# robotics-upo/social_force_window_planner

Measured on AMD Instinct MI355X. Metric: scored trajectories/sec (v x w samples x steps) @ N pedestrians; cmd_vel match, higher is better.
Workload: dtype f64

## Files before the change

include/sfw_hip.h:

```cpp
#ifndef SFW_HIP_H_
#define SFW_HIP_H_

#include <stdint.h>

#ifdef __cplusplus
extern "C" {
#endif

#define SFW_ABI_VERSION 2

typedef enum sfw_status {
  SFW_OK = 0,
  SFW_ERR_INVALID_ARG = -1,
  SFW_ERR_NO_DEVICE = -2,
  SFW_ERR_HIP = -3,
  SFW_ERR_STATE = -4,
  SFW_ERR_UNSUPPORTED = -5
} sfw_status;

#define SFW_COST_INVALID (-1.0)
#define SFW_COST_SKIPPED (-2.0)

#define SFW_ROBOT_ID_NONE INT32_MIN

// ... 69 lines not shown
typedef struct sfw_planner_s *sfw_handle;

void sfw_params_default(sfw_params *p);
int sfw_abi_version(void);
int sfw_create(const sfw_params *params, int device, sfw_handle *out);
int sfw_destroy(sfw_handle h);
int sfw_set_params(sfw_handle h, const sfw_params *params);
const char *sfw_last_error(sfw_handle h);

int sfw_set_costmap(sfw_handle h, const uint8_t *cells, uint32_t size_x,
                    uint32_t size_y, double origin_x, double origin_y,
                    double resolution);
int sfw_set_footprint(sfw_handle h, const double *xy, int32_t K);
int sfw_set_agents(sfw_handle h, const sfw_agent *agents, int32_t A,
                   const double *obstacles_xy, int32_t O);

int sfw_score_grid(sfw_handle h, const sfw_robot_state *rs,
                   const double *linvels, int32_t nv, const double *angvels,
                   int32_t nw, const sfw_goal_args *args, double *costs_out,
                   sfw_best *best_out);

int sfw_score_one(sfw_handle h, const sfw_robot_state *rs, double vx_samp,
                  double vy_samp, double vtheta_samp, const sfw_goal_args *args,
                  double *cost_out, double *points_xyth, int32_t points_cap,
                  int32_t *n_points);

int sfw_grid_stage(sfw_handle h, const sfw_robot_state *rs,
                   const double *linvels, int32_t nv, const double *angvels,
                   int32_t nw, const sfw_goal_args *args, int64_t index_base);
int sfw_grid_launch(sfw_handle h);
int sfw_grid_sync(sfw_handle h);
int sfw_grid_fetch(sfw_handle h, double *costs_out, sfw_best *best_out,
                   sfw_best_key *key_out);
const double *sfw_grid_costs_view(sfw_handle h);

int sfw_samples_stage(sfw_handle h, const sfw_robot_state *rs, const double *vx, const double *vy,
                      const double *vtheta, int32_t n, const sfw_goal_args *args, int64_t index_base);
int sfw_score_samples(sfw_handle h, const sfw_robot_state *rs, const double *vx, const double *vy,
                      const double *vtheta, int32_t n, const sfw_goal_args *args, double *costs_out,
                      sfw_best *best_out);

#define SFW_SEQ_MAX_KNOTS 64
int sfw_sequences_stage(sfw_handle h, const sfw_robot_state *rs, const double *vx, const double *vy,
                        const double *vtheta, int32_t n, int32_t K, const int32_t *knot_step,
                        const sfw_goal_args *args, int64_t index_base);
int sfw_score_sequences(sfw_handle h, const sfw_robot_state *rs, const double *vx, const double *vy,
                        const double *vtheta, int32_t n, int32_t K, const int32_t *knot_step,
                        const sfw_goal_args *args, double *costs_out, sfw_best *best_out);

#define SFW_PERTURB_KEEP_NOMINAL 1
#define SFW_PERTURB_NO_VY        2
#define SFW_PERTURB_KEEP_NORMALS 4
typedef struct sfw_perturb {
  uint64_t seed;
  const double *nominal;
  double sigma[3];
  double lo[3], hi[3];
  int32_t flags, reserved;
} sfw_perturb;
int sfw_sequences_perturb_stage(sfw_handle h, const sfw_robot_state *rs, const sfw_perturb *p, int32_t n, int32_t K,
                                const int32_t *knot_step, const sfw_goal_args *args, int64_t index_base);
int sfw_score_perturbed(sfw_handle h, const sfw_robot_state *rs, const sfw_perturb *p, int32_t n, int32_t K,
                        const int32_t *knot_step, const sfw_goal_args *args, double *costs_out, sfw_best *best_out);
int sfw_sequences_knots(sfw_handle h, int64_t first, int64_t count, double *vx_out, double *vy_out, double *vtheta_out);
int sfw_sequences_normals(sfw_handle h, int64_t first, int64_t count, double *z_out);

#define SFW_ORG_NONE 0
#define SFW_ORG_REGISTER_1 1
#define SFW_ORG_REGISTER_2 2
#define SFW_ORG_FLAT 3
typedef struct sfw_plan_info {
  int32_t split_step;
  int32_t levels;
  int32_t chunks;
  int32_t organisation;
  int64_t classes;
  int64_t class_steps;
  int64_t samples;
  int64_t flat_samples;
  int64_t one_launch;
  int64_t rest_noise_unreproduced;
} sfw_plan_info;
int sfw_grid_plan_info(sfw_handle h, sfw_plan_info *out);
int sfw_plan_shared_prefix(const double *linvels, int32_t nv,
                           const double *angvels, int32_t nw, double vx0,
                           double vtheta0, double acc_x, double acc_theta,
                           double sim_time, int32_t num_steps,
                           int32_t n_agents, int32_t *level_ends,
                           int64_t *level_classes, int32_t cap,
                           int32_t *n_levels);
int sfw_plan_axis_classes(const double *targets, int32_t n, double v0, double a_max, double dt, int32_t max_p,
                          int32_t form, int32_t *counts, int32_t *classes, int32_t *n_levels, int32_t *closed_form);
int sfw_plan_row_blocks(const double *linvels, int32_t nv, const double *angvels, int32_t nw, double vx0,
                        double vtheta0, double acc_x, double acc_theta, double sim_time, int32_t num_steps,
                        int32_t n_agents, int32_t R, int32_t *row0);
#define SFW_K2_AUTO (-1)
#define SFW_K2_REGISTER 0
#define SFW_K2_FLAT 1
int sfw_set_k2_form(sfw_handle h, int32_t form);
int sfw_set_timing(sfw_handle h, int32_t enabled);
int sfw_last_launch_ms(sfw_handle h, int32_t which, float *ms_out);
int sfw_last_clock_ghz(sfw_handle h, double *ghz_out);
int sfw_grid_points(sfw_handle h, int64_t index, double *points_xyth,
                    int32_t points_cap, int32_t *n_points);
int sfw_grid_points_batch(sfw_handle h, int64_t first, int64_t count, double *points_xyth, int32_t *n_points);
int sfw_set_points_capture(sfw_handle h, int32_t enabled);
void *sfw_stream(sfw_handle h);

#define SFW_TERM_VEL 0
#define SFW_TERM_DISTANCE 1
#define SFW_TERM_ANGLE 2
#define SFW_TERM_COSTMAP 3
#define SFW_TERM_SOCIAL 4
#define SFW_N_TERMS 5
#define SFW_RESCORE_MAX_K 1024
typedef struct sfw_weights {
  double vel, distance, angle, costmap, social;
} sfw_weights;
int sfw_set_terms_capture(sfw_handle h, int32_t enabled);
int sfw_grid_rescore(sfw_handle h, const sfw_weights *w, int32_t K, sfw_best *best_out, double *costs_out);
int sfw_grid_terms(sfw_handle h, int64_t first, int64_t count, double *terms_out);

#define SFW_BLEND_MAX_L 16
typedef struct sfw_blend_stat {
  double lambda;
  double j_min;
  double eta;
  double sum_w2;
  int64_t n_valid;
  int64_t index_min;
} sfw_blend_stat;
int sfw_grid_blend(sfw_handle h, const double *lambda, int32_t L, const double *bias,
                   sfw_blend_stat *stat_out, double *u_out, double *weights_out);

int sfw_sequences_control_cost(sfw_handle h, double gamma, double *bias_out);
int sfw_grid_blend_control(sfw_handle h, const double *lambda, int32_t L, double gamma, const double *bias,
                           sfw_blend_stat *stat_out, double *u_out, double *weights_out);

#define SFW_MPPI_MAX_ITER 32
typedef struct sfw_mppi {
  int32_t iterations, reserved;
  double lambda;
  double gamma;
} sfw_mppi;
int sfw_mppi_run(sfw_handle h, const sfw_robot_state *rs, const sfw_perturb *p, int32_t n, int32_t K,
                 const int32_t *knot_step, const sfw_goal_args *args, const sfw_mppi *m,
                 sfw_blend_stat *stat_out , double *plans_out , sfw_best *best_out );

int sfw_score_one_crowd(sfw_handle h, const sfw_robot_state *rs, double vx_samp, double vy_samp, double vtheta_samp,
                        const sfw_goal_args *args, double *cost_out, double *state_xyvv, double *work, int32_t *has_goal,
                        int32_t agents, int32_t steps_cap, int32_t *n_steps);
int sfw_grid_crowd(sfw_handle h, int64_t index, double *cost_out, double *state_xyvv, double *work, int32_t *has_goal,
                   int32_t agents, int32_t steps_cap, int32_t *n_steps);

typedef struct sfw_multi_s *sfw_multi_handle;
#define SFW_MULTI_RCCL 0
#define SFW_MULTI_HOST_REDUCE 1
int sfw_multi_create(const sfw_params *params, const int *devices, int32_t R, int32_t exchange,
                     sfw_multi_handle *out);
int sfw_multi_destroy(sfw_multi_handle m);
const char *sfw_multi_last_error(sfw_multi_handle m);
int32_t sfw_multi_ranks(sfw_multi_handle m);
typedef struct sfw_multi_desc {
  int32_t ranks, exchange, communicators, comm_size, rccl_version;
  int32_t devices[64], comm_devices[64];
  char rccl_path[512], rccl_found[64];
// ... 79 lines not shown
```

social_force_window_planner_amd/_abi.py:

```python
import ctypes as C

SFW_OK = 0
SFW_ERR_INVALID_ARG = -1
SFW_ERR_NO_DEVICE = -2
SFW_ERR_HIP = -3
SFW_ERR_STATE = -4
SFW_ERR_UNSUPPORTED = -5

SFW_COST_INVALID = -1.0
SFW_COST_SKIPPED = -2.0

SFW_PRECISION_F64 = 0
SFW_PRECISION_F32 = 1
SFW_PRECISION_F64_STRICT = 2

SFW_K2_AUTO, SFW_K2_REGISTER, SFW_K2_FLAT = -1, 0, 1
SFW_ORG_NONE, SFW_ORG_REGISTER_1, SFW_ORG_REGISTER_2, SFW_ORG_FLAT = 0, 1, 2, 3


class SfwParams(C.Structure):
    _fields_ = [
        ("max_vel_x", C.c_double),
        ("sim_time", C.c_double),
        ("sim_granularity", C.c_double),
# ... 51 lines not shown
        if not hasattr(p, k):
            raise AttributeError(f"sfw_params has no field {k!r}")
        setattr(p, k, v)
    return p


class SfwAgent(C.Structure):
    _fields_ = [
        ("x", C.c_double),
        ("y", C.c_double),
        ("vx", C.c_double),
        ("vy", C.c_double),
        ("goal_x", C.c_double),
        ("goal_y", C.c_double),
        ("goal_radius", C.c_double),
        ("desired_velocity", C.c_double),
        ("radius", C.c_double),
        ("has_goal", C.c_int32),
        ("id", C.c_int32),
        ("group_id", C.c_int32),
        ("reserved", C.c_int32),
    ]


class SfwRobotState(C.Structure):
    _fields_ = [(n, C.c_double) for n in ("x", "y", "theta", "vx", "vy", "vtheta")]


class SfwGoalArgs(C.Structure):
    _fields_ = [(n, C.c_double) for n in ("acc_x", "acc_y", "acc_theta", "wpx", "wpy")]


class SfwBest(C.Structure):
    _fields_ = [
        ("index", C.c_int64),
        ("cost", C.c_double),
        ("vx", C.c_double),
        ("vy", C.c_double),
        ("vtheta", C.c_double),
        ("n_valid", C.c_int64),
    ]

    def as_dict(self):
        return {n: getattr(self, n) for n, _ in self._fields_}


class SfwBestKey(C.Structure):
    _fields_ = [(n, C.c_double) for n in ("cost", "neg_linvel", "abs_angvel", "neg_index")]

    def as_tuple(self):
        return (self.cost, self.neg_linvel, self.abs_angvel, self.neg_index)


class SfwPlanInfo(C.Structure):
    _fields_ = [("split_step", C.c_int32), ("levels", C.c_int32), ("chunks", C.c_int32), ("organisation", C.c_int32),
                ("classes", C.c_int64), ("class_steps", C.c_int64), ("samples", C.c_int64), ("flat_samples", C.c_int64),
                ("one_launch", C.c_int64), ("rest_noise_unreproduced", C.c_int64)]

    def as_dict(self):
        return {"split_step": self.split_step, "levels": self.levels, "chunks": self.chunks, "classes": self.classes,
                "class_steps": self.class_steps, "samples": self.samples, "organisation": self.organisation,
                "flat_samples": self.flat_samples, "one_launch": self.one_launch,
                "rest_noise_unreproduced": self.rest_noise_unreproduced}


EXPORTED_SYMBOLS = (
    "sfw_params_default",
    "sfw_abi_version",
    "sfw_create",
    "sfw_destroy",
    "sfw_set_params",
    "sfw_last_error",
    "sfw_set_costmap",
    "sfw_set_footprint",
    "sfw_set_agents",
    "sfw_score_grid",
    "sfw_score_one",
    "sfw_grid_stage",
    "sfw_grid_launch",
    "sfw_grid_sync",
    "sfw_grid_fetch",
    "sfw_grid_costs_view",
    "sfw_grid_plan_info",
    "sfw_plan_shared_prefix",
    "sfw_plan_row_blocks",
    "sfw_plan_axis_classes",
    "sfw_set_k2_form",
    "sfw_set_timing",
    "sfw_last_launch_ms",
    "sfw_last_clock_ghz",
    "sfw_grid_points",
    "sfw_grid_points_batch",
    "sfw_set_points_capture",
    "sfw_stream",
    "sfw_multi_create",
    "sfw_multi_destroy",
    "sfw_multi_last_error",
    "sfw_multi_describe",
    "sfw_multi_ranks",
    "sfw_multi_rank_handle",
    "sfw_multi_set_params",
    "sfw_multi_set_costmap",
    "sfw_multi_set_footprint",
    "sfw_multi_set_agents",
    "sfw_multi_score_grid",
    "sfw_multi_rank_rows",
    "sfw_multi_last_us",
    "sfw_multi_grid_points",
    "sfw_batch_create",
    "sfw_batch_destroy",
    "sfw_batch_last_error",
    "sfw_batch_size",
    "sfw_batch_member",
    "sfw_batch_launch",
    "sfw_batch_fetch",
    "sfw_batch_score_grid",
    "sfw_batch_describe",
    "sfw_batch_last_us",
    "sfw_set_terms_capture",
    "sfw_grid_rescore",
    "sfw_grid_terms",
    "sfw_ensemble_create",
    "sfw_ensemble_destroy",
    "sfw_ensemble_last_error",
    "sfw_ensemble_size",
    "sfw_ensemble_member",
    "sfw_ensemble_set_params",
    "sfw_ensemble_set_costmap",
    "sfw_ensemble_set_footprint",
    "sfw_ensemble_set_hypothesis",
    "sfw_ensemble_score_grid",
    "sfw_ensemble_aggregate",
    "sfw_ensemble_last_us",
    "sfw_samples_stage",
    "sfw_score_samples",
    "sfw_sequences_stage",
    "sfw_score_sequences",
    "sfw_score_one_crowd",
    "sfw_grid_crowd",
    "sfw_grid_blend",
    "sfw_sequences_perturb_stage",
    "sfw_score_perturbed",
    "sfw_sequences_knots",
    "sfw_sequences_normals",
    "sfw_ensemble_score_sequences",
    "sfw_ensemble_score_perturbed",
    "sfw_ensemble_blend",
    "sfw_sequences_control_cost",
    "sfw_grid_blend_control",
    "sfw_mppi_run",
    "sfw_ensemble_blend_control",
    "sfw_ensemble_mppi_run",
)
SFW_TERM_VEL, SFW_TERM_DISTANCE, SFW_TERM_ANGLE, SFW_TERM_COSTMAP, SFW_TERM_SOCIAL = 0, 1, 2, 3, 4
SFW_N_TERMS = 5
SFW_RESCORE_MAX_K = 1024


class SfwWeights(C.Structure):

    _fields_ = [("vel", C.c_double), ("distance", C.c_double), ("angle", C.c_double), ("costmap", C.c_double),
                ("social", C.c_double)]


SFW_BLEND_MAX_L = 16

# ... 74 lines not shown
```

social_force_window_planner_amd/csrc/sfw_capi.hip:

```cpp

#include "sfw_device.h"

#include <dlfcn.h>
#include <link.h>

#include <algorithm>
#include <chrono>
#include <cmath>
#include <condition_variable>
#include <functional>
#include <mutex>
#include <thread>
#include <cstdio>
#include <cstdlib>
#include <cstring>
#include <limits>
#include <new>
#include <string>
#include <vector>

namespace {

template <typename T> struct dev_buf {
  T *p = nullptr;
// ... 8 lines not shown
    cap = 0;
    size_t want = n + n / 8 + 16;
    hipError_t e = hipMalloc(reinterpret_cast<void **>(&p), want * sizeof(T));
    if (e == hipSuccess) cap = want;
    return e;
  }
  void release() {
    if (p) (void)hipFree(p);
    p = nullptr;
    cap = 0;
  }
};

struct pinned_buf {
  char *p = nullptr;
  size_t cap = 0;
  hipEvent_t done = nullptr;
  bool pending = false;
  pinned_buf() = default;
  pinned_buf(const pinned_buf &) = delete;
  pinned_buf &operator=(const pinned_buf &) = delete;
  hipError_t wait() {
    if (!pending) return hipSuccess;
    pending = false;
    return hipEventSynchronize(done);
  }
  hipError_t reserve(size_t bytes) {
    hipError_t e = wait();
    if (e != hipSuccess) return e;
    if (!done && (e = hipEventCreateWithFlags(&done, hipEventDisableTiming)) != hipSuccess) return e;
    if (bytes <= cap) return hipSuccess;
    if (p) (void)hipHostFree(p);
    p = nullptr;
    cap = 0;
    const size_t want = bytes + bytes / 4 + 256;
    e = hipHostMalloc(reinterpret_cast<void **>(&p), want, hipHostMallocDefault);
    if (e == hipSuccess) cap = want;
    return e;
  }
  hipError_t mark(hipStream_t s) {
    pending = true;
    return hipEventRecord(done, s);
  }
  void release() {
    (void)wait();
    if (p) (void)hipHostFree(p);
    if (done) (void)hipEventDestroy(done);
    p = nullptr;
    cap = 0;
    done = nullptr;
  }
};

struct level_tables {
  int32_t n_row = 0, n_col = 0;
  size_t o_row_rep = 0, o_col_rep = 0;
  size_t o_row_src = 0, o_col_src = 0;
};
struct chunk_plan {
  std::vector<level_tables> lv;
  size_t o_row_cls = 0;
};

struct map_geometry {
  uint32_t size_x, size_y;
  double origin_x, origin_y, resolution;
};

struct agent_set {
  std::vector<char> blob;
  size_t ao_vel = 0, ao_cst = 0, ao_obs = 0, ao_grp = 0, ao_off = 0, ao_mem = 0;
  int A = 0, O = 0, NG = 0, n_grp_mem = 0;
  bool person_pinned = false;
  std::vector<std::pair<int32_t, int32_t>> rest_pairs;
};

}

struct sfw_planner_s {
  struct config {
    int n_cu = SFW_DEFAULT_CUS, n_xcd = SFW_DEFAULT_CUS / SFW_CUS_PER_XCD;
    std::vector<int> prefix_env;
    bool pin_rest_on = true;
    long spin_us = 20000;
    bool arena_direct_on = true;
    size_t mirror_max_bytes = size_t(64) << 20;
    int obs_tasks_force = -1;
    size_t table_budget_bytes = size_t(8) << 30;
    bool owns_streams = true;
    bool batch_member = false;
  } cfg;

  struct switches {
    sfw_params params;
    uint64_t params_epoch = 1;
    int k2_form = SFW_K2_AUTO;
    bool timing = false;
    bool capture_points = false;
    bool capture_terms = false;
  } live;

  struct world_state {
    map_geometry map_new{0, 0, 0, 0, 0};
    bool have_costmap = false;
    bool cells_dirty = false;
    std::vector<double> footprint;
    int K = 0;
    agent_set agents;
  } world;

  struct stage_record {
    bool valid = false;
    std::vector<double> lin, ang;
    int nv = 0, nw = 0;
    sfw_robot_state rs{};
    sfw_goal_args ga{};
    double vy_samp = 0.0;
    int skip_zero = 1;
    int64_t index_base = 0;
    bool list = false;
    std::vector<double> vy;
    int nk = 1;
    std::vector<int32_t> knot_step;
    const int32_t *d_knot_step = nullptr;
    bool perturbed = false, zero_admitted = false, normals_kept = false;
    sfw_perturb_dev pert{};
    int K = 0, A = 0, O = 0, NG = 0, n_grp_mem = 0;
    bool person_pinned = false;
    map_geometry map{0, 0, 0, 0, 0};
    const uint8_t *d_cells = nullptr;
    bool cells_in_arena = false;
    size_t arena_cells_bytes = 0;
    const double *d_footprint = nullptr, *d_agent_pos = nullptr, *d_agent_vel = nullptr, *d_obstacles = nullptr;
    const sfw_agent_const *d_agent_c = nullptr;
    const int32_t *d_agent_grp = nullptr, *d_grp_off = nullptr, *d_grp_mem = nullptr;
    const double *d_linvels = nullptr, *d_angvels = nullptr;
    const double *d_vy = nullptr;
    const double *d_agent_rest = nullptr;
    const double *d_pin_rest = nullptr;
    sfw_sel *d_sel = nullptr;
    std::vector<std::pair<int32_t, int32_t>> rest_pairs;
    std::vector<double> rest_pv;
    size_t pin_doubles = 0;
    std::vector<double> pin_pos;
    std::vector<sfw_agent_const> pin_cst;
    std::vector<int> prefix_steps;
    std::vector<chunk_plan> prefix_chunks;
    size_t prefix_o_col_cls = 0;
    int prefix_S = 0;
    int64_t prefix_chunk = 0;
    int64_t prefix_class_steps = 0, prefix_last_classes = 0;
    std::vector<int32_t> cls_ints;
    int64_t cls_max = 0;
    bool cls_two = false;
    const int32_t *d_cls_tab = nullptr;
    int64_t table_chunk = 0;
    uint64_t plan_epoch = 0;
    bool arena_pending = false;
    size_t arena_from = 0, arena_bytes = 0;
    bool early_poses = false;
    bool early_poses_timed = false;
    bool early_poses_terms = false;
    bool clock_cleared = false;
  } st;

  struct launch_record {
// ... 113 lines not shown
        return e;
      }
      polled = true;
      if (std::chrono::duration_cast<std::chrono::microseconds>(std::chrono::steady_clock::now() - t0).count() > h->cfg.spin_us) break;
#if defined(__x86_64__)
      __builtin_ia32_pause();
#endif
    }
    (void)hipGetLastError();
  }
  return hipStreamSynchronize(h->stream);
}
void stream_is_idle(sfw_handle h) { h->pin_map.pending = h->pin_arena.pending = h->pin_cls.pending = false; }

constexpr int64_t kRowLimit = static_cast<int64_t>((uint64_t(1) << 32) / (2 * sizeof(sfw_unit))) - 2;

int num_steps_of(const sfw_params &p) {
  int n = static_cast<int>(p.sim_time / p.sim_granularity + 0.5);
  return n == 0 ? 1 : n;
}

int check_params(sfw_handle h, const sfw_params *p) {
  if (!p) return fail(h, SFW_ERR_INVALID_ARG, "params is NULL");
  if (!(p->sim_granularity > 0) || !(p->sim_time >= 0))
    return fail(h, SFW_ERR_INVALID_ARG, "sim_time/sim_granularity out of range");
  if (p->precision != SFW_PRECISION_F64 && p->precision != SFW_PRECISION_F32 && p->precision != SFW_PRECISION_F64_STRICT)
    return fail(h, SFW_ERR_INVALID_ARG, "unknown precision");
  if (!(p->sfm_gamma > 0) || !(p->sfm_relaxation_time > 0) || !(p->sfm_force_sigma_obstacle > 0))
    return fail(h, SFW_ERR_INVALID_ARG, "sfm gamma/relaxation_time/sigma must be > 0");
  if (!(p->sfm_force_factor_social >= 0) || !(p->sfm_force_factor_obstacle >= 0))
    return fail(h, SFW_ERR_INVALID_ARG, "sfm_force_factor_social / _obstacle must be >= 0");
  return SFW_OK;
}

int64_t table_row_units(int64_t stride, int nw) { return stride + stride / (nw > 0 ? nw : 1) + 2; }
constexpr size_t kTableBytesPerSampleStep = sizeof(sfw_unit) + sizeof(int16_t);

void fill_launch(sfw_handle h, sfw_launch &L, int64_t begin, int64_t count, int64_t stride) {
  std::memset(&L, 0, sizeof(L));
  L.p = h->live.params;
  L.S = num_steps_of(h->live.params);
  L.dt = h->live.params.sim_time / L.S;
  L.rs = h->st.rs;
  L.ga = h->st.ga;
  L.vy_samp = h->st.vy_samp;
  L.skip_zero_sample = h->st.skip_zero;
  L.linvels = h->st.d_linvels;
  L.angvels = h->st.d_angvels;
  L.nv = h->st.nv;
  L.nw = h->st.nw;
  L.vy_samps = h->st.d_vy;
  L.list = h->st.list ? 1 : 0;
  L.n_knots = h->st.nk;
  L.knot_step = h->st.d_knot_step;
  L.knot_stride = h->st.nv;
  L.chunk_begin = begin;
  L.chunk_count = count;
  L.cells = h->st.d_cells;
  L.size_x = h->st.map.size_x;
  L.size_y = h->st.map.size_y;
  L.origin_x = h->st.map.origin_x;
  L.origin_y = h->st.map.origin_y;
  L.resolution = h->st.map.resolution;
  L.footprint = h->st.d_footprint;
  L.K = h->st.K;
  L.agent_pos = h->st.d_agent_pos;
  L.agent_vel = h->st.d_agent_vel;
  L.agent_c = h->st.d_agent_c;
  L.agent_rest = h->st.d_agent_rest;
  L.pin_rest = h->st.d_pin_rest;
  L.A = h->st.A;
  L.obstacles = h->st.d_obstacles;
  L.O = h->st.O;
  L.agent_grp = h->st.d_agent_grp;
  L.grp_off = h->st.d_grp_off;
  L.grp_mem = h->st.d_grp_mem;
  L.NG = h->st.NG;
  L.n_grp_mem = h->st.n_grp_mem;
  L.n_cu = h->cfg.n_cu;
  L.n_xcd = h->cfg.n_xcd;
  sfw_derive(L);
  if (h->cfg.obs_tasks_force >= 0 && L.O > 0) L.k.obs_tasks = h->cfg.obs_tasks_force;
  L.pair_tab = h->pair_tab.p;
  L.status = h->status.p;
  L.base_cost = h->base_cost.p;
  L.costs = h->costs.p;
  L.coll_step = h->coll_step.p;
  L.ptab = h->ptab.p;
  L.cs_tab = h->cs_tab.p;
  L.row_units = table_row_units(stride, h->st.nw);
  L.fcode = h->fcode.p;
  L.rstep_stride = stride;
  L.points = nullptr;
  L.n_points = nullptr;
  L.phase = SFW_PHASE_WHOLE;
  L.step_begin = 0;
  L.step_end = L.S;
  L.resume = 0;
  L.k2_form = h->live.k2_form;
  L.index_base = h->st.index_base;
  L.cycle_counter = h->cycle_counter.p;
  L.sel_out = h->st.d_sel;
  L.costs_host = nullptr;
  L.sel_host = nullptr;
  L.arena_host = nullptr;
  L.arena_dev = nullptr;
  L.arena_bytes = 0;
}

double new_velocity_host(double vg, double vi, double a_max, double dt) {
  if ((vg - vi) >= 0) return std::fmin(vg, vi + a_max * dt);
  return std::fmax(vg, vi - a_max * dt);
}

void velocity_classes(const std::vector<double> &targets, double v0, double a_max, double dt, int max_p,
                      std::vector<std::vector<int32_t>> &cls, std::vector<int32_t> &counts) {
  const size_t n = targets.size();
  std::vector<int32_t> order(n);
  for (size_t i = 0; i < n; ++i) order[i] = static_cast<int32_t>(i);
  std::sort(order.begin(), order.end(), [&](int32_t a, int32_t b) {
    return targets[static_cast<size_t>(a)] != targets[static_cast<size_t>(b)] ? targets[static_cast<size_t>(a)] < targets[static_cast<size_t>(b)]
                                                                                : a < b;
  });
  std::vector<double> t(n), v(n, v0);
  for (size_t k = 0; k < n; ++k) t[k] = targets[static_cast<size_t>(order[k])];
  std::vector<int32_t> cur(n, 0), nxt(n);
  cls.clear();
  counts.clear();
  for (int p = 0; p < max_p; ++p) {
    int32_t id = -1;
    uint64_t prev_bits = 0;
    for (size_t k = 0; k < n; ++k) {
      v[k] = new_velocity_host(t[k], v[k], a_max, dt);
      uint64_t bits;
      std::memcpy(&bits, &v[k], sizeof(bits));
      if (k == 0 || cur[k] != cur[k - 1] || bits != prev_bits) ++id;
      nxt[k] = id;
      prev_bits = bits;
    }
    cur.swap(nxt);
    cls.emplace_back(n);
    std::vector<int32_t> &out = cls.back();
    for (size_t k = 0; k < n; ++k) out[static_cast<size_t>(order[k])] = cur[k];
    counts.push_back(id + 1);
    if (static_cast<size_t>(id + 1) == n) break;
  }
}

double step_cost(double items, double items_per_wave, int cus) {
  const double capacity = 4.0 * cus * 5.5;
  const double x = items / items_per_wave / capacity;
  return x <= 1.0 ? 0.45 + 0.55 * x : x;
}

struct axis_classes {
  std::vector<int32_t> n;
  std::vector<double> targets;
  double v0 = 0, a_max = 0, dt = 0;
  int max_p = 0;
  bool made_for(const std::vector<double> &t, double v0_, double a_, double dt_, int mp) const {
    return v0 == v0_ && a_max == a_ && dt == dt_ && max_p == mp && targets == t;
  }
  const std::vector<int32_t> &level(int p) const {
    const size_t l = std::min<size_t>(static_cast<size_t>(p), n.size()) - 1;
    if (!fast) return c[l];
    if (c[l].empty()) write_level(l);
// ... 1221 lines not shown
                                         const_cast<double *>(h->st.d_angvels), h->st.normals_kept ? h->normals.p : nullptr, h->stream));
    }
    if (int e = launch_common(h)) return e;
    const double *d_bias = nullptr;
    if (m->gamma != 0.0) {
      if (int e = control_cost_enqueue(h, m->gamma, nullptr, plan, h->ctrl_bias, h->blend_bias)) return e;
      d_bias = h->ctrl_bias.p;
    }
    if (int e = blend_enqueue(h, area, h->costs.p, n, K, h->st.d_linvels, h->st.d_vy, h->st.d_angvels, 1, true, &m->lambda, 1, d_bias,
                              nullptr, pin + i * slot, plan))
      return e;
  }
  SFW_HIP(h, h->pin_mppi.mark(h->stream));
  sfw_best best;
  if (int e = sfw_grid_fetch(h, nullptr, &best, nullptr)) return e;
  h->pin_mppi.pending = false;
  for (int i = 0; i < I; ++i) blend_finish(pin + i * slot, &m->lambda, 1, K, stat_out + i, plans_out + static_cast<size_t>(i) * 3 * K);
  if (I > 1) std::memcpy(h->st.pert.nominal, plans_out + static_cast<size_t>(I - 2) * 3 * K, plan_bytes);
  if (best_out) *best_out = best;
  return SFW_OK;
}
}

extern "C" {

void sfw_params_default(sfw_params *p) {
  if (!p) return;
  std::memset(p, 0, sizeof(*p));
  p->max_vel_x = 0.7;
  p->sim_time = 1.0;
  p->sim_granularity = 0.025;
  p->robot_radius = 0.35f;
  p->social_weight = 1.2;
  p->costmap_weight = 2.0;
  p->angle_weight = 0.7;
  p->distance_weight = 1.0;
  p->vel_weight = 1.0;
  p->robot_goal_radius = 0.20;
  p->sfm_force_factor_desired = 2.0;
  p->sfm_force_factor_obstacle = 10.0;
  p->sfm_force_sigma_obstacle = 0.2;
  p->sfm_force_factor_social = 2.1;
  p->sfm_lambda = 2.0;
  p->sfm_gamma = 0.35;
  p->sfm_n = 2.0;
  p->sfm_n_prime = 3.0;
  p->sfm_relaxation_time = 0.5;
  p->sfm_force_factor_group_gaze = 3.0;
  p->sfm_force_factor_group_coherence = 2.0;
  p->sfm_force_factor_group_repulsion = 1.0;
  p->precision = SFW_PRECISION_F64;
}

int sfw_abi_version(void) { return SFW_ABI_VERSION; }

}

namespace {
int destroy_handle(sfw_handle h);
int create_handle(const sfw_params *params, int device, hipStream_t stream, hipStream_t side, sfw_handle *out) {
  if (!out) return SFW_ERR_INVALID_ARG;
  *out = nullptr;
  if (int e = check_params(nullptr, params)) return e;
  int count = 0;
  if (hipGetDeviceCount(&count) != hipSuccess || count <= 0) return SFW_ERR_NO_DEVICE;
  if (device < 0 || device >= count) return SFW_ERR_INVALID_ARG;
  sfw_handle h = new (std::nothrow) sfw_planner_s();
  if (!h) return SFW_ERR_HIP;
  h->live.params = *params;
  h->device = device;
  if (const char *b = std::getenv("SFW_PREFIX")) {
    for (const char *q = b; *q;) {
      char *end = nullptr;
      const long v = std::strtol(q, &end, 10);
      if (end == q) break;
      if (v >= 0) h->cfg.prefix_env.push_back(static_cast<int>(v));
      q = (*end == ',') ? end + 1 : end;
    }
    std::sort(h->cfg.prefix_env.begin(), h->cfg.prefix_env.end());
    h->cfg.prefix_env.erase(std::unique(h->cfg.prefix_env.begin(), h->cfg.prefix_env.end()), h->cfg.prefix_env.end());
  }
  if (const char *b = std::getenv("SFW_FORCE_FLAT")) h->live.k2_form = std::atoi(b) == 1 ? SFW_K2_FLAT : std::atoi(b) == 0 ? SFW_K2_REGISTER : SFW_K2_AUTO;
  if (const char *b = std::getenv("SFW_PIN_REST")) h->cfg.pin_rest_on = std::atoi(b) != 0;
  if (const char *b = std::getenv("SFW_SPIN_US")) h->cfg.spin_us = std::max(0L, std::atol(b));
  if (const char *b = std::getenv("SFW_ARENA_DIRECT")) h->cfg.arena_direct_on = std::atoi(b) != 0;
  if (const char *b = std::getenv("SFW_MIRROR_MAX_MB")) h->cfg.mirror_max_bytes = static_cast<size_t>(std::max(0L, std::atol(b))) << 20;
  if (const char *b = std::getenv("SFW_OBS_TASKS")) h->cfg.obs_tasks_force = std::atoi(b) != 0 ? 1 : 0;
  if (const char *b = std::getenv("SFW_TABLE_BUDGET_MB")) {
    long mb = std::atol(b);
    if (mb > 0) h->cfg.table_budget_bytes = static_cast<size_t>(mb) << 20;
  }
  hipError_t e = hipSetDevice(device);
  if (e == hipSuccess) {
    hipDeviceProp_t prop;
    if (hipGetDeviceProperties(&prop, device) == hipSuccess && prop.multiProcessorCount > 0) h->cfg.n_cu = prop.multiProcessorCount;
    h->cfg.n_cu = env_device_cus(h->cfg.n_cu);
    int xccs = 0;
    if (!std::getenv("SFW_DEVICE_CUS") && hipDeviceGetAttribute(&xccs, hipDeviceAttributeNumberOfXccs, device) == hipSuccess && xccs >= 1)
      h->cfg.n_xcd = xccs;
    else
      h->cfg.n_xcd = std::max(1, h->cfg.n_cu / SFW_CUS_PER_XCD);
    (void)hipGetLastError();
    if (const char *b = std::getenv("SFW_DEVICE_XCDS")) {
      const long v = std::atol(b);
      if (v >= 1 && v <= 64) h->cfg.n_xcd = static_cast<int>(v);
    }
  }
  if (stream) {
    h->cfg.owns_streams = false;
    h->stream = stream;
    h->side = side;
  } else {
    if (e == hipSuccess) e = hipStreamCreateWithFlags(&h->stream, hipStreamNonBlocking);
    if (e == hipSuccess) e = hipStreamCreateWithFlags(&h->side, hipStreamNonBlocking);
  }
  if (e == hipSuccess) e = hipEventCreateWithFlags(&h->ev_poses, hipEventDisableTiming);
  if (e == hipSuccess) e = hipEventCreateWithFlags(&h->ev_side, hipEventDisableTiming);
  if (e == hipSuccess) e = hipEventCreateWithFlags(&h->split.fork, hipEventDisableTiming);
  if (e == hipSuccess) e = hipEventCreateWithFlags(&h->split.join, hipEventDisableTiming);
  if (e == hipSuccess) h->split.side = h->side;
  for (int i = 0; i < 5 && e == hipSuccess; ++i) e = hipEventCreate(&h->ev[i]);
  if (e == hipSuccess) e = h->cycle_counter.reserve(1);
  if (e == hipSuccess) e = hipMemsetAsync(h->cycle_counter.p, 0, sizeof(unsigned), h->stream);
  if (e != hipSuccess) {
    destroy_handle(h);
    return SFW_ERR_HIP;
  }
  *out = h;
  return SFW_OK;
}

int destroy_handle(sfw_handle h) {
  (void)hipSetDevice(h->device);
  if (h->stream) (void)hipStreamSynchronize(h->stream);
  if (h->side) (void)hipStreamSynchronize(h->side);
  h->cells.release();
  h->arena.release();
  h->pair_tab.release();
  h->crowd_pair_tab.release();
  h->crowd_out.release();
  h->pin_crowd.release();
  h->status.release();
  h->coll_step.release();
  h->base_cost.release();
  h->costs.release();
  h->ptab.release();
  h->cs_tab.release();
  h->fcode.release();
  h->partials.release();
  h->clock.release();
  h->cycle_counter.release();
  h->pin_cap.release();
  h->terms.release();
  h->rescore_w.release();
  h->rescore_partials.release();
  h->rescore_costs.release();
  h->pin_rescore.release();
  h->blend_mins.release();
  h->blend_partials.release();
  h->blend_bias.release();
  h->blend_weights.release();
  h->pin_blend.release();
  h->ctrl_bias.release();
  h->mppi_plan.release();
  h->pin_mppi.release();
  h->normals.release();
// ... 407 lines not shown
    std::memcpy(points_xyth, h->pin_out.p + head, sizeof(double) * 3 * static_cast<size_t>(m));
  }
  return SFW_OK;
}

int sfw_plan_shared_prefix(const double *linvels, int32_t nv, const double *angvels, int32_t nw, double vx0, double vtheta0,
                           double acc_x, double acc_theta, double sim_time, int32_t num_steps, int32_t n_agents,
                           int32_t *level_ends, int64_t *level_classes, int32_t cap, int32_t *n_levels) {
  if (!linvels || !angvels || nv <= 0 || nw <= 0 || num_steps < 1 || !n_levels || cap < 0 ||
      (cap > 0 && (!level_ends || !level_classes)))
    return SFW_ERR_INVALID_ARG;
  *n_levels = 0;
  const int64_t T = static_cast<int64_t>(nv) * nw;
  if (n_agents < 2 || num_steps < 2 || T < 4096) return SFW_OK;
  const std::vector<double> lin(linvels, linvels + nv), ang(angvels, angvels + nw);
  prefix_classes pc;
  classes_of_grid(pc, lin, ang, vx0, vtheta0, acc_x, acc_theta, sim_time / num_steps, num_steps);
  const int cus = env_device_cus(SFW_DEFAULT_CUS);
  const std::vector<int> steps = choose_levels(pc, T, num_steps, static_cast<double>(sfw_samples_per_wave(n_agents, T, SFW_K2_AUTO, cus)), cus);
  *n_levels = static_cast<int32_t>(steps.size());
  for (size_t l = 0; l < steps.size() && l < static_cast<size_t>(cap); ++l) {
    level_ends[l] = steps[l];
    level_classes[l] = static_cast<int64_t>(pc.n_rows_at(steps[l])) * pc.n_cols_at(steps[l]);
  }
  return SFW_OK;
}

int sfw_plan_axis_classes(const double *targets, int32_t n, double v0, double a_max, double dt, int32_t max_p, int32_t form,
                          int32_t *counts, int32_t *classes, int32_t *n_levels, int32_t *closed_form) {
  if (!targets || n <= 0 || max_p < 1 || !counts || !n_levels || (form != 0 && form != 1)) return SFW_ERR_INVALID_ARG;
  if (!all_finite(targets, static_cast<size_t>(n)) || !std::isfinite(v0) || !std::isfinite(a_max) || !std::isfinite(dt))
    return SFW_ERR_INVALID_ARG;
  const axis_classes a = classes_of_axis(std::vector<double>(targets, targets + n), v0, a_max, dt, max_p, form == 0);
  *n_levels = static_cast<int32_t>(a.n.size());
  if (closed_form) *closed_form = a.fast ? 1 : 0;
  for (size_t l = 0; l < a.n.size(); ++l) {
    counts[l] = a.n[l];
    if (classes) std::memcpy(classes + l * static_cast<size_t>(n), a.level(static_cast<int>(l) + 1).data(), sizeof(int32_t) * static_cast<size_t>(n));
  }
  return SFW_OK;
}

int sfw_plan_row_blocks(const double *linvels, int32_t nv, const double *angvels, int32_t nw, double vx0, double vtheta0,
                        double acc_x, double acc_theta, double sim_time, int32_t num_steps, int32_t n_agents, int32_t R,
                        int32_t *row0) {
  if (!linvels || !angvels || nv <= 0 || nw <= 0 || num_steps < 1 || R < 1 || !row0) return SFW_ERR_INVALID_ARG;
  if (!all_finite(linvels, static_cast<size_t>(nv)) || !all_finite(angvels, static_cast<size_t>(nw))) return SFW_ERR_INVALID_ARG;
  const std::vector<double> lin(linvels, linvels + nv), ang(angvels, angvels + nw);
  std::vector<int32_t> cuts;
  plan_row_blocks(lin, ang, vx0, vtheta0, acc_x, acc_theta, sim_time / num_steps, num_steps, n_agents, R, SFW_K2_AUTO,
                  env_device_cus(SFW_DEFAULT_CUS), cuts);
  std::memcpy(row0, cuts.data(), sizeof(int32_t) * (static_cast<size_t>(R) + 1));
  return SFW_OK;
}

int sfw_grid_plan_info(sfw_handle h, sfw_plan_info *out) {
  if (!h || !out) return SFW_ERR_INVALID_ARG;
  if (!h->st.valid) return fail(h, SFW_ERR_STATE, "grid_plan_info before grid_stage");
  const int64_t T = static_cast<int64_t>(h->st.nv) * h->st.nw;
  out->split_step = h->st.prefix_steps.empty() ? 0 : h->st.prefix_steps.back();
  out->levels = static_cast<int32_t>(h->st.prefix_steps.size());
  out->samples = T;
  out->classes = h->st.prefix_last_classes;
  out->class_steps = h->st.prefix_class_steps;
  if (!h->st.prefix_steps.empty()) {
    out->chunks = static_cast<int32_t>(h->st.prefix_chunks.size());
  } else {
    int64_t chunk = h->st.table_chunk;
    if (chunk > T) chunk = T;
    out->chunks = chunk > 0 ? static_cast<int32_t>((T + chunk - 1) / chunk) : 0;
  }
  out->organisation = sfw_social_organisation(h->st.A, out->chunks > 0 ? (T + out->chunks - 1) / out->chunks : T, h->st.O, h->live.k2_form, h->cfg.n_cu);
  out->flat_samples = sfw_social_flat_items(h->st.A, h->st.O, h->st.NG, out->chunks > 0 ? (T + out->chunks - 1) / out->chunks : T, h->live.k2_form, h->cfg.n_cu);
  out->rest_noise_unreproduced = rest_noise_unreproduced(h) ? 1 : 0;
  out->one_launch = 0;
  if (out->chunks == 1 && h->st.prefix_steps.empty()) {
    sfw_launch L;
    fill_launch(h, L, 0, T, T);
    out->one_launch = sfw_cycle_applies(L) ? 1 : 0;
  }
  return SFW_OK;
}

int sfw_set_k2_form(sfw_handle h, int32_t form) {
  if (!h) return SFW_ERR_INVALID_ARG;
  if (form != SFW_K2_AUTO && form != SFW_K2_REGISTER && form != SFW_K2_FLAT)
    return fail(h, SFW_ERR_INVALID_ARG, "set_k2_form: form must be SFW_K2_AUTO, SFW_K2_REGISTER or SFW_K2_FLAT");
  h->live.k2_form = form;
  return SFW_OK;
}

int sfw_set_timing(sfw_handle h, int32_t enabled) {
  if (!h) return SFW_ERR_INVALID_ARG;
  h->live.timing = enabled != 0;
  return SFW_OK;
}

int sfw_last_launch_ms(sfw_handle h, int32_t which, float *ms_out) {
  if (!h || !ms_out) return SFW_ERR_INVALID_ARG;
  if (!h->last.launched) return fail(h, SFW_ERR_STATE, "last_launch_ms before grid_launch");
  if (!h->last.timed) return fail(h, SFW_ERR_STATE, "last_launch_ms: timing was off for the last launch (sfw_set_timing)");
  SFW_HIP(h, hipSetDevice(h->device));
  SFW_HIP(h, hipEventSynchronize(h->ev[3]));
  if (h->last.n_chunks > 1 && (which == 1 || which == 2)) {
    float total = 0.0f;
    for (int c = 0; c < h->last.n_chunks; ++c) {
      float ms = 0.0f;
      const int a = 3 * c + (which == 1 ? 0 : 1);
      SFW_HIP(h, hipEventElapsedTime(&ms, h->chunk_ev[a], h->chunk_ev[a + 1]));
      total += ms;
    }
    *ms_out = total;
    return SFW_OK;
  }
  int a = 0, b = 3;
  switch (which) {
    case 0: a = 0; b = 3; break;
    case 1: a = 0; b = 1; break;
    case 2: a = 1; b = 2; break;
    case 3: a = 2; b = 3; break;
    default: return fail(h, SFW_ERR_INVALID_ARG, "last_launch_ms: which must be 0..3");
  }
  SFW_HIP(h, hipEventElapsedTime(ms_out, h->ev[a], h->ev[b]));
  return SFW_OK;
}

int sfw_set_points_capture(sfw_handle h, int32_t enabled) {
  if (!h) return SFW_ERR_INVALID_ARG;
  h->live.capture_points = enabled != 0;
  return SFW_OK;
}

int sfw_set_terms_capture(sfw_handle h, int32_t enabled) {
  if (!h) return SFW_ERR_INVALID_ARG;
  h->live.capture_terms = enabled != 0;
  if (!h->live.capture_terms) {
    h->last.terms = false;
    h->st.early_poses_terms = false;
    if (h->terms.p) {
      SFW_HIP(h, hipSetDevice(h->device));
      SFW_HIP(h, hipStreamSynchronize(h->stream));
      h->terms.release();
    }
  }
  return SFW_OK;
}

int sfw_grid_rescore(sfw_handle h, const sfw_weights *w, int32_t K, sfw_best *best_out, double *costs_out) {
  if (!h) return SFW_ERR_INVALID_ARG;
  if (!w || !best_out) return fail(h, SFW_ERR_INVALID_ARG, "grid_rescore: weights or best_out is NULL");
  if (K < 1 || K > SFW_RESCORE_MAX_K) return fail(h, SFW_ERR_INVALID_ARG, "grid_rescore: K out of [1, SFW_RESCORE_MAX_K]");
  if (!all_finite(reinterpret_cast<const double *>(w), static_cast<size_t>(K) * SFW_N_TERMS))
    return fail(h, SFW_ERR_INVALID_ARG, "grid_rescore: non-finite weight");
  if (!h->last.launched || !h->last.terms)
    return fail(h, SFW_ERR_STATE, "grid_rescore: the last launch did not capture terms (sfw_set_terms_capture), or a stage or "
                                  "sfw_score_one came in since");
  SFW_HIP(h, hipSetDevice(h->device));
  const int64_t T = static_cast<int64_t>(h->st.nv) * h->st.nw;
  const size_t sel_bytes = (sizeof(sfw_sel) * static_cast<size_t>(K) + 15) & ~size_t(15);
  const size_t w_bytes = sizeof(sfw_weights) * static_cast<size_t>(K);
  if (sel_bytes + w_bytes > h->pin_rescore.cap) SFW_HIP(h, hipStreamSynchronize(h->stream));
  SFW_HIP(h, h->pin_rescore.reserve(sel_bytes + w_bytes));
  sfw_sel *const sel_host = reinterpret_cast<sfw_sel *>(h->pin_rescore.p);
  std::memcpy(h->pin_rescore.p + sel_bytes, w, w_bytes);
  SFW_HIP(h, h->rescore_w.reserve(static_cast<size_t>(K)));
  SFW_HIP(h, hipMemcpyAsync(h->rescore_w.p, h->pin_rescore.p + sel_bytes, w_bytes, hipMemcpyHostToDevice, h->stream));
// ... 1555 lines not shown
```

social_force_window_planner_amd/csrc/sfw_device.h:

```cpp
#ifndef SFW_DEVICE_H_
#define SFW_DEVICE_H_

#include <hip/hip_runtime.h>
#include <stdint.h>

#include "../../include/sfw_hip.h"


#define SFW_DEFAULT_CUS 256
#define SFW_CUS_PER_XCD 32

enum : int32_t { SFW_ST_VALID = 0, SFW_ST_INVALID = 1, SFW_ST_SKIPPED = 2 };

struct __attribute__((aligned(32))) sfw_robot_step {
  double x, y, vx, vy;
};

struct __attribute__((aligned(32))) sfw_pose_frame {
  double x, y, c, s;
};

struct __attribute__((aligned(16))) sfw_unit {
  double a, b;
};
// ... 40 lines not shown
  double cost;
  double neg_linvel;
  double abs_angvel;
  long long neg_index;
  long long n_valid;
};

struct sfw_launch {
  sfw_params p;
  sfw_derived k;
  int32_t S;
  double dt;
  sfw_robot_state rs;
  sfw_goal_args ga;
  double vy_samp;
  int32_t skip_zero_sample;
  const double *linvels;
  const double *angvels;
  int32_t nv, nw;
  int64_t chunk_begin;
  int64_t chunk_count;
  const uint8_t *cells;
  uint32_t size_x, size_y;
  double origin_x, origin_y, resolution;
  const double *footprint;
  int32_t K;
  const double *agent_pos;
  const double *agent_vel;
  const sfw_agent_const *agent_c;
  const double *agent_rest;
  const double *pin_rest;
  int32_t A;
  const double *obstacles;
  int32_t O;
  const int32_t *agent_grp;
  const int32_t *grp_off;
  const int32_t *grp_mem;
  int32_t NG;
  int32_t n_grp_mem;
  int32_t phase;
  int32_t step_begin, step_end;
  int32_t resume;
  int32_t force_alive;
  int32_t k2_form;
  int32_t n_cu, n_xcd;
  int32_t n_cls, n_col_cls;
  int32_t item_base;
  const int32_t *row_rep;
  const int32_t *col_rep;
  int32_t n_col_src;
  const int32_t *row_src, *col_src;
  const sfw_cls_agent *in_state;
  const int32_t *in_dead;
  sfw_cls_agent *out_state;
  int32_t *out_dead;
  const uint16_t *pair_tab;
  int32_t *status;
  double *base_cost;
  double *costs;
  int32_t *coll_step;
  sfw_unit *ptab;
  sfw_unit *cs_tab;
  int64_t row_units;
  int16_t *fcode;
  int64_t rstep_stride;
  double *points;
  int32_t *n_points;
  unsigned long long *clock_probe;
  int64_t index_base;
  unsigned *cycle_counter;
  sfw_sel *sel_out;
  double *costs_host;
  sfw_sel *sel_host;
  const char *arena_host;
  char *arena_dev;
  uint32_t arena_bytes;
  double *terms;
  int64_t terms_T;
  const double *vy_samps;
  int32_t list;
  int32_t n_knots;
  const int32_t *knot_step;
  int64_t knot_stride;
};

__device__ __forceinline__ void sfw_put_term(double *terms, int64_t T, int64_t t, int k, double v) {
  if (terms) terms[k * T + t] = v;
}
__device__ __forceinline__ void sfw_put_terms3(double *terms, int64_t T, int64_t t, double vel, double d, double ang) {
  if (!terms) return;
  terms[SFW_TERM_VEL * T + t] = vel;
  terms[SFW_TERM_DISTANCE * T + t] = d;
  terms[SFW_TERM_ANGLE * T + t] = ang;
}
__device__ __forceinline__ void sfw_put_terms_sentinel(double *terms, int64_t T, int64_t t, double sentinel) {
  if (!terms) return;
  for (int k = 0; k < SFW_N_TERMS; ++k) terms[k * T + t] = sentinel;
}


struct sfw_crowd_out {
  double *state;
  double *work;
  int32_t *has_goal;
};

void sfw_derive(sfw_launch &L);

hipError_t sfw_launch_rollout(const sfw_launch &L, hipStream_t stream);
hipError_t sfw_launch_rollout_poses(const sfw_launch &L, hipStream_t stream);
hipError_t sfw_launch_rollout_costmap(const sfw_launch &L, hipStream_t stream);
struct sfw_split_streams {
  hipStream_t side;
  hipEvent_t fork, join;
};
hipError_t sfw_launch_social(const sfw_launch &L, hipStream_t stream, const sfw_split_streams *sp = nullptr);
bool sfw_cycle_applies(const sfw_launch &L);
hipError_t sfw_launch_cycle(const sfw_launch &L, hipStream_t stream);
struct sfw_batch_rec {
  sfw_launch L;
  int32_t k2_bytes;
  int32_t lds_bytes;
};
inline size_t sfw_batch_recs_offset(int B) { return (sizeof(uint32_t) * (static_cast<size_t>(B) + 1) + 15) & ~size_t(15); }
int sfw_cycle_batch_variant(const sfw_launch &L);
void sfw_cycle_batch_record(const sfw_launch &L, sfw_batch_rec *rec);
hipError_t sfw_launch_cycle_batch(int variant, const uint32_t *d_first, const sfw_batch_rec *d_recs, int B, unsigned blocks,
                                  size_t lds, hipStream_t stream);
#ifndef SFW_STRICT_BUILD
hipError_t sfw_launch_cycle_batch_strict(int variant, const uint32_t *d_first, const sfw_batch_rec *d_recs, int B,
                                         unsigned blocks, size_t lds, hipStream_t stream);
int64_t sfw_social_flat_items(int A, int O, int NG, int64_t T, int form, int cus);
hipError_t sfw_launch_social_strict(const sfw_launch &L, hipStream_t stream, const sfw_split_streams *sp = nullptr);
hipError_t sfw_launch_cycle_strict(const sfw_launch &L, hipStream_t stream);
hipError_t sfw_launch_crowd_strict(const sfw_launch &L, const sfw_crowd_out &cw, hipStream_t stream);
#endif
hipError_t sfw_launch_crowd(const sfw_launch &L, const sfw_crowd_out &cw, hipStream_t stream);
bool sfw_rollout_is_fused(const sfw_launch &L);
int64_t sfw_argmin_partials(int64_t T);
hipError_t sfw_launch_argmin(const double *costs, const double *linvels, const double *angvels,
                             int32_t nw, int64_t T, int64_t index_base, sfw_sel *partials,
                             sfw_sel *out, hipStream_t stream, double *costs_host = nullptr,
                             sfw_sel *sel_host = nullptr, bool list = false);
int64_t sfw_rescore_blocks(int64_t T, int K);
hipError_t sfw_launch_rescore(const double *terms, int64_t T, const sfw_weights *w, int K, const double *linvels,
                              const double *angvels, int32_t nw, int64_t index_base, sfw_sel *partials, double *costs,
                              sfw_sel *sel_host, hipStream_t stream, bool list = false);
hipError_t sfw_launch_ensemble(const double *const *terms, const double *probs, int M, int64_t T, int mode, const sfw_weights &w,
                               const double *linvels, const double *angvels, int32_t nw, double *costs, int32_t *rejected,
                               sfw_sel *partials, sfw_sel *sel_host, hipStream_t stream);
hipError_t sfw_launch_ensemble_list(const double *const *terms, const double *probs, int M, int64_t T, int mode,
                                    const sfw_weights &w, const double *linvels, const double *angvels, double *costs,
                                    double *costs_dev, int32_t *rejected, sfw_sel *partials, sfw_sel *sel_host, hipStream_t stream);
struct sfw_blend_min {
  double j;
  int64_t index;
  int64_t n_valid;
};
struct sfw_blend_lambdas {
  double v[SFW_BLEND_MAX_L];
};
int64_t sfw_blend_blocks(int64_t T);
int64_t sfw_blend_min_blocks(int64_t T);
inline int64_t sfw_blend_channels(int L, int K) { return 2 * static_cast<int64_t>(L) + 3 * static_cast<int64_t>(K) * L; }
hipError_t sfw_launch_blend(const double *costs, const double *bias, int64_t T, const sfw_blend_lambdas &lam, int L, int K,
                            const double *linvels, const double *vy, const double *angvels, int32_t nw, bool list,
                            sfw_blend_min *mins, double *partials, double *weights, sfw_blend_min *min_host, double *out_host,
                            hipStream_t stream, double *plan = nullptr);
hipError_t sfw_launch_blend_weights(const double *costs, const double *bias, int64_t T, const sfw_blend_lambdas &lam, int L,
                                    const sfw_blend_min *mins, double *weights, hipStream_t stream);
struct sfw_perturb_dev {
  uint32_t key0, key1;
  int32_t keep_nominal, pad;
  double sigma[3], lo[3], hi[3];
  double nominal[SFW_SEQ_MAX_KNOTS * 3];
};
hipError_t sfw_launch_perturb(const sfw_perturb_dev &a, int64_t n, int K, int64_t index_base, double *vx, double *vy, double *vtheta,
                              double *z_out, hipStream_t stream);
struct sfw_perturb_head {
  uint32_t key0, key1;
  int32_t keep_nominal, pad;
  double sigma[3], lo[3], hi[3];
};
static_assert(sizeof(sfw_perturb_head) == offsetof(sfw_perturb_dev, nominal), "sfw_perturb_head is the head of sfw_perturb_dev");
hipError_t sfw_launch_perturb_plan(const sfw_perturb_dev &a, const double *plan, int64_t n, int K, int64_t index_base, double *vx,
                                   double *vy, double *vtheta, double *z_out, hipStream_t stream);
struct sfw_perturb_dst {
  double *vx, *vy, *vtheta, *z;
};
hipError_t sfw_launch_perturb_members(const sfw_perturb_dev &a, const double *plan, int64_t n, int K, int64_t index_base,
                                      const sfw_perturb_dst *dst, int M, hipStream_t stream);
hipError_t sfw_launch_control_cost(const sfw_perturb_dev &a, const double *plan, int K, int64_t n, int64_t index_base,
                                   const double *z_kept, double gamma, const double *bias_add, double *bias, hipStream_t stream);
hipError_t sfw_launch_key_table(const sfw_sel *sel, double *table, int r, int R, hipStream_t stream);
int64_t sfw_pair_table_entries(int A);
hipError_t sfw_launch_pair_table(uint16_t *tab, int A, hipStream_t stream, bool runtime_cap = false);
int sfw_samples_per_wave(int A, int64_t T, int form, int cus);
size_t sfw_social_lds_bytes(int A, int O, int NG, int n_grp_mem, int64_t T, int form, int cus);
int sfw_social_organisation(int A, int64_t T, int O, int form, int cus);

#endif
```

social_force_window_planner_amd/csrc/sfw_kernels.hip:

```cpp

#include "sfw_device.h"
#include "sfw_math.h"

#include <type_traits>

#include <limits.h>
#include <math.h>
#include <stdlib.h>
#include <cmath>

namespace {

constexpr int WAVE = 64;

#pragma clang fp contract(off)

__device__ __forceinline__ unsigned cell_index(double a, double res, double inv_res) {
  const double q = a * inv_res;
  const double m = __builtin_trunc(q);
  const double d = q - m;
  if (d < 1e-9 || d > 1.0 - 1e-9) return static_cast<unsigned>(a / res);
  return static_cast<unsigned>(m);
}

// ... 606 lines not shown
    if (tid == 0 && L.n_points) L.n_points[q.local] = 0;
    return;
  }
  k1s_footprint(L, a, S, tid, nthr);
  __syncthreads();
  k1s_quotients(a, S, tid, nthr);
  __syncthreads();
  if (tid == 0) k1s_scan(L, a, q, S);
}

#pragma clang fp contract(fast)

template <typename R> struct tiny_of;
template <> struct tiny_of<double> { static constexpr double v = 1e-300; };
template <> struct tiny_of<float> { static constexpr float v = 1e-30f; };

__device__ __forceinline__ unsigned xcd_contiguous(unsigned b, unsigned n, unsigned nx) {
  nx = nx ? nx : 1u;
  const unsigned x = b % nx, k = b / nx;
  const unsigned q = n / nx, r = n % nx;
  return x * q + (x < r ? x : r) + k;
}

typedef const __attribute__((address_space(4))) sfw_launch *late_launch;
__device__ __forceinline__ late_launch late_args() {
  const __attribute__((address_space(4))) void *p =
      (const __attribute__((address_space(4))) void *)__builtin_amdgcn_kernarg_segment_ptr();
  asm volatile("" : "+s"(p));
  return static_cast<late_launch>(p);
}
template <bool BATCH> __device__ __forceinline__ late_launch late_args_of(late_launch rec) {
  if constexpr (!BATCH) {
    (void)rec;
    return late_args();
  } else {
    const __attribute__((address_space(4))) void *p = rec;
    asm volatile("" : "+s"(p));
    return static_cast<late_launch>(p);
  }
}

__device__ __forceinline__ void clock_probe(int which) {
  if (blockIdx.x != gridDim.x / 2 || threadIdx.x != 0) return;
  unsigned long long *const p = late_args()->clock_probe;
  if (!p) return;
  p[2 * which] = __builtin_readcyclecounter();
  p[2 * which + 1] = wall_clock64();
}

template <typename R> struct sfm_consts {
  sfwm::poly_consts pc;
  R lambda, neg_l2e_inv_gamma, l2_f_social, c_vel, c_ang;
};
struct agent_consts {
  double f_desired, inv_tau, dt, rr, inv_O, l2_f_obstacle, l2e_inv_sigma;
  double f_gaze, f_coherence, f_repulsion;
  const double *obstacles;
  int O, robot_id, obs_tasks;
};
__device__ __forceinline__ agent_consts load_agent_consts(late_launch La, bool f32) {
  agent_consts c;
  c.f_desired = La->k.f_desired;
  c.inv_tau = La->k.inv_tau;
  c.dt = La->dt;
  c.rr = La->k.rr;
  c.inv_O = La->k.inv_O;
  c.l2_f_obstacle = f32 ? static_cast<double>(La->k.f.l2_f_obstacle) : La->k.d.l2_f_obstacle;
  c.l2e_inv_sigma = f32 ? static_cast<double>(La->k.f.l2e_inv_sigma) : La->k.d.l2e_inv_sigma;
  c.f_gaze = La->p.sfm_force_factor_group_gaze;
  c.f_coherence = La->p.sfm_force_factor_group_coherence;
  c.f_repulsion = La->p.sfm_force_factor_group_repulsion;
  c.O = La->O;
  c.obstacles = La->obstacles;
  c.obs_tasks = La->k.obs_tasks;
  c.robot_id = La->agent_c[0].id;
  return c;
}

__device__ __forceinline__ double copysign_from(double mag, double sgn) { return __builtin_copysign(mag, sgn); }
__device__ __forceinline__ float copysign_from(float mag, double sgn) {
  return __builtin_copysignf(mag, static_cast<float>(sgn));
}

template <typename R, bool NORM_ONLY = false>
__device__ __forceinline__ void pair_force(const sfm_consts<R> &k, R dx, R dy, R wx, R wy, double cw, R &fx,
                                           R &fy) {
  using namespace sfwm;
  const R tiny = tiny_of<R>::v;
  R rd, dn, rl, il;
  const R d2 = fma(dx, dx, fma(dy, dy, tiny));
  rsqrt_sqrt(d2, rd, dn);
  const R ux = dx * rd, uy = dy * rd;
  const R ix = fma(k.lambda, wx, ux), iy = fma(k.lambda, wy, uy);
  const R l2 = fma(ix, ix, fma(iy, iy, tiny));
  rsqrt_sqrt(l2, rl, il);
  const R sn = fma(ix, uy, -(iy * ux));
  const R ncs = fma(-ix, ux, -(iy * uy));
  const R theta = angle_abs(k.pc, fabs(sn), ncs, rl, il);
  const R a = fmax(fma(dn * rl, k.neg_l2e_inv_gamma, k.l2_f_social), R(-1100));
  const R t2 = l2 * (theta * theta);
  R ev, ea;
  exp2_fast2_gated(k.pc, fma(k.c_vel, t2, a), fma(k.c_ang, t2, a), cw, ev, ea);
  if constexpr (NORM_ONLY) {
    const R q = fma(ev, ev, ea * ea);
    R rq, nq;
    rsqrt_sqrt(fma(R(1), q, tiny), rq, nq);
    fx = q * rq;
    fy = R(0);
    return;
  }
  ea = copysign_from(ea, cw);
  const R gx = ix * rl, gy = iy * rl;
  fx = fma(ea, gy, -(ev * gx));
  fy = fma(-ev, gy, -(ea * gx));
}
template <typename R, bool NORM_ONLY = false>
__device__ __forceinline__ void pair_force_state(const sfm_consts<R> &k, double pix, double piy, double vix,
                                                 double viy, double pjx, double pjy, double vjx, double vjy,
                                                 R &fx, R &fy) {
  const double dx = pjx - pix, dy = pjy - piy, wx = vix - vjx, wy = viy - vjy;
  const double cw = fma(wx, dy, -(wy * dx));
  pair_force<R, NORM_ONLY>(k, R(dx), R(dy), R(wx), R(wy), cw, fx, fy);
}

__device__ __forceinline__ double fast_norm(double x, double y) {
  const double q = fma(x, x, y * y);
  double rs, sq;
  sfwm::rsqrt_sqrt(fmax(q, 1e-300), rs, sq);
  return q * rs;
}

__device__ __forceinline__ double scaled_norm(double x, double y) {
  const double m = fmax(fabs(x), fabs(y));
  if (!(m > 0.0)) return 0.0;
  const int e = __builtin_amdgcn_frexp_exp(m);
  const double sx = __builtin_amdgcn_ldexp(x, -e), sy = __builtin_amdgcn_ldexp(y, -e);
  double rs, sq;
  sfwm::rsqrt_sqrt(fma(sx, sx, sy * sy), rs, sq);
  return __builtin_amdgcn_ldexp(sq, e);
}

__device__ __forceinline__ void desired_force(const agent_consts &k, double px, double py, double vx, double vy,
                                              bool has_goal, double gx, double gy, double gr, double dv, double &fx,
                                              double &fy) {
  const double ex = gx - px, ey = gy - py;
  double inv, en;
  sfwm::rsqrt_sqrt(fmax(fma(ex, ex, ey * ey), 1e-300), inv, en);
  if (has_goal && en > gr) {
    fx = k.f_desired * (ex * inv * dv - vx) * k.inv_tau;
    fy = k.f_desired * (ey * inv * dv - vy) * k.inv_tau;
  } else {
    fx = -vx * k.inv_tau;
    fy = -vy * k.inv_tau;
  }
}

constexpr int OBS_SEG = 16;
constexpr int OBS_AGENT_LANES = WAVE / OBS_SEG;
constexpr int OBS_AGENTS_PER_LANE = 4;
typedef const __attribute__((address_space(4))) double *obs_global_ptr;
__device__ __forceinline__ obs_global_ptr obs_global(const double *obstacles) {
  return (obs_global_ptr)(const __attribute__((address_space(1))) double *)obstacles;
}
__device__ __forceinline__ double2 obs_point(const double2 *obs, int o) { return obs[o]; }
__device__ __forceinline__ double2 obs_point(obs_global_ptr obs, int o) { return double2{obs[2 * o], obs[2 * o + 1]}; }
template <typename R>
__device__ __forceinline__ void obstacle_term(const sfm_consts<R> &k, double2 q, double px, double py, R nis, R &ax, R &ay) {
  using namespace sfwm;
  const R mx = R(px - q.x), my = R(py - q.y);
  R rm, mn;
  rsqrt_sqrt(fma(mx, mx, fma(my, my, tiny_of<R>::v)), rm, mn);
  const R e = exp2_scaled(k.pc, mn, nis) * rm;
  ax = fma(e, mx, ax);
  ay = fma(e, my, ay);
}
template <typename R, typename ObsPtr>
__device__ __forceinline__ void obstacle_segment(const sfm_consts<R> &k, ObsPtr obs, int o_begin, int o_end,
                                                 double px, double py, R nis, R &ax, R &ay) {
  ax = R(0);
  ay = R(0);
#pragma unroll 4
  for (int o = o_begin; o < o_end; ++o) obstacle_term<R>(k, obs_point(obs, o), px, py, nis, ax, ay);
}
typedef const __attribute__((address_space(3))) double *obs_lds_ptr;
__device__ __forceinline__ double2 obs_point(obs_lds_ptr obs, int o) { return double2{obs[2 * o], obs[2 * o + 1]}; }
typedef double obs_d2 __attribute__((ext_vector_type(2)));
__device__ __forceinline__ obs_d2 obs_load_ahead(const double2 *base, uint32_t lane_bytes) {
  obs_d2 q;
  asm volatile("s_nop 4\n\tglobal_load_dwordx4 %0, %1, %2" : "=v"(q) : "v"(lane_bytes), "s"(base) : "memory");
  return q;
}
template <int YOUNGER> __device__ __forceinline__ void obs_load_wait(obs_d2 &q) {
  asm volatile("s_waitcnt vmcnt(%1)" : "+v"(q) : "n"(YOUNGER));
}
template <typename R, int NJ>
__device__ __forceinline__ void obstacle_segment_multi_uniform(const sfm_consts<R> &k, obs_lds_ptr obs, int O, int Lseg, int seg,
                                                               const double *px, const double *py, R neg_l2e_inv_sigma, R *ax,
                                                               R *ay) {
#pragma unroll
  for (int j = 0; j < NJ; ++j) ax[j] = ay[j] = R(0);
  const R nis = neg_l2e_inv_sigma;
  auto terms = [&](const double2 q) {
#pragma unroll
    for (int j = 0; j < NJ; ++j) obstacle_term<R>(k, q, px[j], py[j], nis, ax[j], ay[j]);
  };
// ... 9 lines not shown
      terms(qa);
      terms(qb);
      qa = qn;
    }
    if (i < n) terms(qa);
  };
  const int first = partial > 0 ? partial : Lseg;
  if (seg < n_full + (partial > 0 ? 1 : 0)) run(mine, first);
  if (first < Lseg && seg < n_full) run(mine + 2 * first, Lseg - first);
}
template <typename R, int NJ>
__device__ __forceinline__ void obstacle_segment_multi_uniform(const sfm_consts<R> &k, const double2 *obs, int O, int Lseg, int seg,
                                                               const double *px, const double *py, R neg_l2e_inv_sigma, R *ax,
                                                               R *ay) {
#pragma unroll
  for (int j = 0; j < NJ; ++j) ax[j] = ay[j] = R(0);
  const R nis = neg_l2e_inv_sigma;
  auto terms = [&](const obs_d2 q) {
#pragma unroll
    for (int j = 0; j < NJ; ++j) obstacle_term<R>(k, double2{q.x, q.y}, px[j], py[j], nis, ax[j], ay[j]);
  };
  const int n_full = O / Lseg, partial = O - n_full * Lseg;
  const uint32_t lane_bytes = static_cast<uint32_t>(seg * Lseg) * 16u;
  auto run = [&](const double2 *base, int n) {
    obs_d2 qa = obs_load_ahead(base, lane_bytes);
    int i = 0;
#pragma unroll 1
    for (; i + 2 <= n; i += 2) {
      obs_d2 qb = obs_load_ahead(base + i + 1, lane_bytes);
      obs_load_wait<1>(qa);
      terms(qa);
      qa = obs_load_ahead(base + i + 2, lane_bytes);
      obs_load_wait<1>(qb);
      terms(qb);
    }
    obs_load_wait<0>(qa);
    if (i < n) terms(qa);
  };
  const int first = partial > 0 ? partial : Lseg;
  if (seg < n_full + (partial > 0 ? 1 : 0)) run(obs, first);
  if (first < Lseg && seg < n_full) run(obs + first, Lseg - first);
}
template <typename R>
__device__ __forceinline__ double obstacle_scale(const sfm_consts<R> &k, const agent_consts &c, double radius) {
  return static_cast<double>(sfwm::exp2_fast(k.pc, static_cast<R>(fma(radius, c.l2e_inv_sigma, c.l2_f_obstacle)))) * c.inv_O;
}
template <typename R>
__device__ __forceinline__ void obstacle_sums(const sfm_consts<R> &k, const agent_consts &c, obs_global_ptr obs, double px,
                                              double py, double radius, double &tx_out, double &ty_out, double &scale) {
  const int O = c.O, L = (O + OBS_SEG - 1) / OBS_SEG;
  const R nis = sfwm::vgpr_const(static_cast<R>(-c.l2e_inv_sigma));
  R tx = R(0), ty = R(0);
  R ax = R(0), ay = R(0);
  for (int b = 0; b < O; b += L) {
    obstacle_segment<R, obs_global_ptr>(k, obs, b, min(b + L, O), px, py, nis, ax, ay);
    tx += ax;
    ty += ay;
  }
  tx_out = static_cast<double>(tx);
  ty_out = static_cast<double>(ty);
  scale = obstacle_scale<R>(k, c, radius);
}

__device__ __forceinline__ double swap_pair(double v) {
  const uint64_t u = __builtin_bit_cast(uint64_t, v);
  constexpr int QP_1032 = 0xB1;
  const uint32_t lo = static_cast<uint32_t>(__builtin_amdgcn_update_dpp(0, static_cast<int>(static_cast<uint32_t>(u)), QP_1032, 0xf, 0xf, true));
  const uint32_t hi = static_cast<uint32_t>(__builtin_amdgcn_update_dpp(0, static_cast<int>(static_cast<uint32_t>(u >> 32)), QP_1032, 0xf, 0xf, true));
  return __builtin_bit_cast(double, (static_cast<uint64_t>(hi) << 32) | lo);
}

struct lds_layout {
  double *px, *py, *vx, *vy, *fjx, *fjy, *fcx, *fcy;
  double2 *gcen;
  double2 *obs;
  sfw_robot_step *rsb;
  sfw_agent_const *ac;
  double *swp;
  double2 *opart;
  double *wr;
  double *oscale;
  int *hasgoal, *dead, *grp, *goff, *gmem;
  unsigned char *hasgoal8;
  int hg_stride;
  size_t bytes;
  static constexpr int REG_DEAD_CAP = 32;
  __host__ __device__ lds_layout(char *base, int A, int cap, int GA, int G, int O, int NG, int NM, bool consts,
                                 bool with_frc, bool obs_in_lds = false) {
    char *const base0 = base;
    auto take = [&](size_t n) {
      char *p = base;
      base += (n + 15) & ~size_t(15);
      return p;
    };
    const size_t plane = sizeof(double) * static_cast<size_t>(cap);
    px = reinterpret_cast<double *>(take(plane));
    py = reinterpret_cast<double *>(take(plane));
    vx = reinterpret_cast<double *>(take(plane));
    vy = reinterpret_cast<double *>(take(plane));
    fjx = reinterpret_cast<double *>(take(plane));
    fjy = reinterpret_cast<double *>(take(plane));
    if (with_frc) {
      fcx = reinterpret_cast<double *>(take(plane));
      fcy = reinterpret_cast<double *>(take(plane));
      rsb = reinterpret_cast<sfw_robot_step *>(take(sizeof(sfw_robot_step) * 2));
      swp = reinterpret_cast<double *>(take(sizeof(double) * GA));
      opart = reinterpret_cast<double2 *>(take(sizeof(double2) * (O > 0 ? (obs_in_lds ? 4 : 2) * 64 : 0)));
      wr = reinterpret_cast<double *>(take(sizeof(double) * (O > 0 ? 4 : 0)));
      oscale = reinterpret_cast<double *>(take(sizeof(double) * (O > 0 ? A : 0)));
      obs = reinterpret_cast<double2 *>(take(sizeof(double2) * (obs_in_lds ? O + 2 : 0)));
      if (!obs_in_lds) obs = nullptr;
      hasgoal8 = reinterpret_cast<unsigned char *>(take(static_cast<size_t>(GA)));
      hasgoal = nullptr;
      hg_stride = 1;
      dead = reinterpret_cast<int *>(take(sizeof(int) * G));
    } else {
      fcx = fcy = nullptr;
      opart = nullptr;
      wr = nullptr;
      oscale = nullptr;
      obs = nullptr;
      hasgoal = reinterpret_cast<int *>(take(plane));
      hasgoal8 = nullptr;
      hg_stride = 2;
      swp = reinterpret_cast<double *>(take(plane));
      dead = reinterpret_cast<int *>(take(sizeof(int) * REG_DEAD_CAP));
      rsb = reinterpret_cast<sfw_robot_step *>(take(sizeof(sfw_robot_step) * G));
    }
    ac = reinterpret_cast<sfw_agent_const *>(take(sizeof(sfw_agent_const) * (consts ? A : 0)));
    gcen = reinterpret_cast<double2 *>(take(sizeof(double2) * (NG > 0 ? G * NG : 0)));
    grp = reinterpret_cast<int *>(take(sizeof(int) * (NG > 0 ? A : 0)));
    goff = reinterpret_cast<int *>(take(sizeof(int) * (NG > 0 ? NG + 1 : 0)));
    gmem = reinterpret_cast<int *>(take(sizeof(int) * (NG > 0 && NM > 0 ? NM : 0)));
    bytes = static_cast<size_t>(base - base0);
  }
  __device__ __forceinline__ int hg(int sl) const { return hg_stride == 1 ? static_cast<int>(hasgoal8[sl]) : hasgoal[sl * hg_stride]; }
};
template <int CAP> struct reg_off {
  static constexpr int PY = 8 * CAP, VX = 16 * CAP, VY = 24 * CAP, FJX = 32 * CAP, FJY = 40 * CAP, HG = 48 * CAP, SW = 56 * CAP,
                       DEAD = 64 * CAP, RSB = 64 * CAP + 4 * lds_layout::REG_DEAD_CAP;
};

struct agent_k {
  double gx, gy, gr, dv, rad;
  int id;
};
__device__ __forceinline__ agent_k agent_k_of(const sfw_agent_const &c) {
  return agent_k{c.goal_x, c.goal_y, c.goal_radius, c.desired_velocity, c.radius, c.id};
}
__device__ __forceinline__ agent_k agent_k_lds(const lds_layout &s, int i) { return agent_k_of(s.ac[i]); }
__device__ __forceinline__ agent_k agent_k_global(const sfw_agent_const *agent_c, int i) { return agent_k_of(agent_c[i]); }

template <typename R>
__device__ double2 group_force(const sfm_consts<R> &k, const agent_consts &c, const lds_layout &s, int NG, int g, int A,
                               int i, int sl, double px, double py) {
  const sfw_agent_const ci = s.ac[i];
  const int q = s.grp[i];
  if (q < 0) return double2{0.0, 0.0};
  const int m0 = s.goff[q], m1 = s.goff[q + 1];
  if (m1 - m0 < 2) return double2{0.0, 0.0};
  const double n = static_cast<double>(m1 - m0), inv_n = sfwm::rcp_nr(n);
  const double2 csum = s.gcen[g * NG + q];
  const double cx = csum.x * inv_n, cy = csum.y * inv_n;
  const double ex = ci.goal_x - px, ey = ci.goal_y - py;
  double inv_en, en;
  sfwm::rsqrt_sqrt(fmax(fma(ex, ex, ey * ey), 1e-300), inv_en, en);
  const bool has_dir = s.hg(sl) && en > ci.goal_radius;
  const double ddx = has_dir ? ex * inv_en : 0.0, ddy = has_dir ? ey * inv_en : 0.0;
  double fx = 0.0, fy = 0.0;
  {
    const double w = sfwm::rcp_nr(n - 1.0);
    const double rx = fma(w, fma(n, cx, -px), -px), ry = fma(w, fma(n, cy, -py), -py);
    const double ep = fma(ddx, rx, ddy * ry);
    if (ep < 0.0) {
      const double sc = c.f_gaze * ep;
      fx = sc * ddx;
      fy = sc * ddy;
    }
  }
  {
    const double rx = cx - px, ry = cy - py;
    const double dist = fast_norm(rx, ry);
    const double x2 = fmin(2.0 * ((n - 1.0) * 0.5 - dist), 700.0);
    const double soft = c.f_coherence * sfwm::rcp_nr(1.0 + sfwm::exp2_fast(k.pc, x2 * 1.4426950408889634074));
    fx = fma(rx, soft, fx);
    fy = fma(ry, soft, fy);
  }
  double rx = 0.0, ry = 0.0;
  const double ra = ci.radius;
  for (int m = m0; m < m1; ++m) {
    const int b = s.gmem[m];
    if (b == i) continue;
    const double dx = px - s.px[g * A + b], dy = py - s.py[g * A + b], rr = ra + s.ac[b].radius;
    if (fma(dx, dx, dy * dy) < rr * rr) { rx += dx; ry += dy; }
  }
  fx = fma(rx, c.f_repulsion, fx);
  fy = fma(ry, c.f_repulsion, fy);
  return double2{fx, fy};
}

template <typename R> __device__ __forceinline__ const sfw_force_k<R> &force_k(const sfw_launch &L);
template <> __device__ __forceinline__ const sfw_force_k<double> &force_k<double>(const sfw_launch &L) { return L.k.d; }
template <> __device__ __forceinline__ const sfw_force_k<float> &force_k<float>(const sfw_launch &L) { return L.k.f; }

template <typename R, bool PIN_ALL> __device__ __forceinline__ sfm_consts<R> make_consts(const sfw_launch &L) {
  const sfw_force_k<R> &f = force_k<R>(L);
  sfm_consts<R> k;
  k.lambda = sfwm::vgpr_const(f.lambda);
  k.neg_l2e_inv_gamma = sfwm::vgpr_const(f.neg_l2e_inv_gamma);
  k.l2_f_social = PIN_ALL ? sfwm::vgpr_const(f.l2_f_social) : f.l2_f_social;
  k.c_vel = sfwm::vgpr_const(f.c_vel);
  k.c_ang = PIN_ALL ? sfwm::vgpr_const(f.c_ang) : f.c_ang;
  return k;
}

template <typename R, bool PIN_ALL> __device__ __forceinline__ sfm_consts<R> make_consts(late_launch La) {
// ... 420 lines not shown
            sw[r] += lds_at<double>(smem, io + off::SW) + fast_norm(tx * sc, ty * sc);
            const sfw_robot_step r2 = lds_at<sfw_robot_step>(smem, off::RSB + 8u * g4_[r]);
            lds_at<double>(smem, io) = r2.x;
            lds_at<double>(smem, io + PY) = r2.y;
            lds_at<double>(smem, io + VX) = r2.vx;
            lds_at<double>(smem, io + VY) = r2.vy;
          } else {
            fx[r] = fma(tx, sc, fx[r]);
            fy[r] = fma(ty, sc, fy[r]);
          }
        }
    }
    if (const double *const pin = late_args()->pin_rest) {
#pragma unroll
      for (int r = 0; r < NS; ++r)
        if (ok_[r] && lds_at<int>(smem, off::DEAD + g4_[r]) == 0 &&
            pin_at_rest(pin, lds_at<sfw_robot_step>(smem, off::RSB + 8u * g4_[r]))) {
          const int i = lds_at<int2>(smem, io_[r] + off::HG).y >> 1;
          if (i == 0) {
            fx[r] += pin[2];
            fy[r] += pin[3];
          } else {
            sw[r] += pin[4 + i];
          }
        }
    }
    __syncthreads();
    bool any_live = false;
    for (int g = 0; g < G; ++g) any_live |= (s.dead[g] == 0);
    if (!any_live) break;
    if constexpr (GROUPS) add_group_forces(k, c);
      }

  const late_launch Le = late_args();
  if (Le->phase == SFW_PHASE_PREFIX) {
    sfw_cls_agent *const out_state = Le->out_state;
    const int64_t A_late = Le->A;
#pragma unroll
    for (int r = 0; r < NS; ++r)
      if (ok_[r] && static_cast<int>(g4_[r] >> 2) < Gn) {
        const uint32_t io = io_[r];
        sfw_cls_agent c;
        c.px = lds_at<double>(smem, io); c.py = lds_at<double>(smem, io + PY);
        c.vx = lds_at<double>(smem, io + VX); c.vy = lds_at<double>(smem, io + VY);
        c.fx = fx[r]; c.fy = fy[r]; c.sw = sw[r];
        const int2 cell = lds_at<int2>(smem, io + off::HG);
        c.hasgoal = cell.x;
        c.pad = 0;
        out_state[(first_local + static_cast<int64_t>(g4_[r] >> 2)) * A_late + (cell.y >> 1)] = c;
      }
    if (lane < Gn) Le->out_dead[first_local + lane] = s.dead[lane];
    clock_probe(1);
    return;
  }
  double sw_acc = 0.0;
#pragma unroll
  for (int r = 0; r < NS; ++r) {
    if (G == 1) sw_acc += ok_[r] ? sw[r] : 0.0;
    else if (ok_[r]) lds_at<double>(smem, io_[r] + off::SW) = sw[r];
  }
  finish_wave(s, lane, G, Gn, first_local, sw_acc);
  clock_probe(1);
}
template <typename R, int NS, bool GROUPS>
__global__ void __launch_bounds__(WAVE, (NS == 1 && !GROUPS) ? 6 : 1) sfw_social_kernel(const sfw_launch L, const int G) {
  sfwm::fp_mode_for_omod();
  extern __shared__ __attribute__((aligned(16))) char smem[];
  social_reg_wave<R, NS, GROUPS>(L, G, smem, blockIdx.x, gridDim.x);
}

__global__ void __launch_bounds__(256) sfw_pair_table_kernel(uint16_t *tab, int A, int n_entries, int n_dummy) {
  const int u = blockIdx.x * blockDim.x + threadIdx.x;
  if (u >= n_entries) return;
  const int P = A * (A - 1) / 2;
  int i = A + (u >= P ? (u - P) % n_dummy : 0), j = i;
  if (u < P) {
    const int row = u / A;
    i = u - row * A;
    j = i + row + 1;
    j = (j >= A) ? j - A : j;
  }
  tab[u] = static_cast<uint16_t>(8 * i);
  tab[n_entries + u] = static_cast<uint16_t>(8 * j);
}

__device__ __forceinline__ void load_pair_entries(const uint16_t *ti, const uint16_t *tj, uint32_t lane_off, uint32_t &io,
                                                  uint32_t &jo) {
  asm volatile("s_nop 4\n\tglobal_load_ushort %0, %2, %3\n\tglobal_load_ushort %1, %2, %4"
               : "=&v"(io), "=&v"(jo)
               : "v"(lane_off), "s"(ti), "s"(tj));
}
__device__ __forceinline__ void wait_pair_entries(uint32_t &io, uint32_t &jo) {
  asm volatile("s_waitcnt vmcnt(0)" : "+v"(io), "+v"(jo));
}

#ifndef SFW_FLAT_WAVES
#define SFW_FLAT_WAVES 5
#endif
#ifndef SFW_FLAT_WAVES_NOOBS
#define SFW_FLAT_WAVES_NOOBS 6
#endif
__device__ __forceinline__ void wave_sync() {
  __builtin_amdgcn_fence(__ATOMIC_RELEASE, "wavefront");
  __builtin_amdgcn_wave_barrier();
  __builtin_amdgcn_fence(__ATOMIC_ACQUIRE, "wavefront");
}
struct cycle_result {
  double social_work;
  int dead;
  int ready;
  int fdone;
  int legal;
  double base0, base;
};
__device__ __forceinline__ int cycle_wait_ready(const cycle_result *res, int need) {
  int r;
  while ((r = *const_cast<const volatile int *>(&res->ready)) < need) __builtin_amdgcn_s_sleep(1);
  __builtin_amdgcn_fence(__ATOMIC_ACQUIRE, "workgroup");
  return r;
}
#define K2_SYNC() do { if constexpr (CYCLE) wave_sync(); else __syncthreads(); } while (0)
template <typename R, bool GROUPS, int CAP, bool OBS, bool CYCLE, bool BATCH = false, bool CAPTURE = false>
__device__ __forceinline__ void social_flat_wave(const sfw_launch &L, char *const smem, const k1s_lds *const k1, cycle_result *const res,
                                                 const unsigned bid, const unsigned nblk, const int64_t item_base,
                                                 const late_launch Lb = nullptr, const sfw_crowd_out cw = sfw_crowd_out{}) {
  static_assert(CYCLE || !BATCH, "a batched wave is a cycle kernel's wave");
  static_assert(!CAPTURE || (!CYCLE && !BATCH), "the crowd capture runs as a kernel of its own");
  const int lane = threadIdx.x;
  const int A = L.A, O = L.O;
  const int NG = GROUPS ? L.NG : 0;
  const int cap = CAP > 0 ? CAP : ((A + 2) & ~1);
  const int PY = 8 * cap, VX = 16 * cap, VY = 24 * cap, FJX = 32 * cap, FJY = 40 * cap, FCX = 48 * cap,
            FCY = 56 * cap;
  (void)FCX;
  (void)FCY;
  constexpr bool CONSTS_IN_LDS = GROUPS || CYCLE;
  const lds_layout s(smem, A, cap, A, 1, O, NG, GROUPS ? L.n_grp_mem : 0, CONSTS_IN_LDS, true, L.k.obs_lds != 0);
  const int64_t first_local = CYCLE ? static_cast<int64_t>(bid) : item_base + xcd_contiguous(bid, nblk, static_cast<unsigned>(L.n_xcd));
  const sfm_consts<R> k0 = make_consts<R, true>(L);
  const sfw_force_k<R> &fk = force_k<R>(L);
  const R s_lambda = sfwm::sgpr_const(fk.lambda), s_nig = sfwm::sgpr_const(fk.neg_l2e_inv_gamma), s_lfs = sfwm::sgpr_const(fk.l2_f_social),
          s_cvel = sfwm::sgpr_const(fk.c_vel), s_cang = sfwm::sgpr_const(fk.c_ang);
  constexpr bool F32 = sizeof(R) == 4;
  const int step_begin = L.step_begin, step_end = L.step_end;
  if constexpr (CYCLE) {
    stage_consts<GROUPS, CONSTS_IN_LDS>(L, s, lane);
    if (lane == 0) s.dead[0] = 0;
    wave_sync();
  } else {
    if (!stage_wave<GROUPS, GROUPS>(L, s, lane, 1, 1, first_local)) {
      if (L.phase == SFW_PHASE_SUFFIX) finish_wave(s, lane, 1, 1, first_local, 0.0);
      if (L.phase == SFW_PHASE_PREFIX && lane == 0) L.out_dead[first_local] = s.dead[0];
      return;
    }
  }
  if constexpr (!BATCH) clock_probe(0);
  const int64_t rsample_v = CYCLE ? 0 : robot_sample_of_item(L, first_local);
  const int64_t rsample = static_cast<int64_t>(
      (static_cast<uint64_t>(static_cast<uint32_t>(__builtin_amdgcn_readfirstlane(static_cast<int>(rsample_v >> 32)))) << 32) |
      static_cast<uint32_t>(__builtin_amdgcn_readfirstlane(static_cast<int>(rsample_v))));

  if (!CYCLE && L.resume) {
    const sfw_cls_agent *rec = L.in_state + source_class_of_item(L, first_local) * A;
    for (int sl = lane; sl < A; sl += WAVE) {
      const sfw_cls_agent c = rec[sl];
      s.px[sl] = c.px;
      s.py[sl] = c.py;
      s.vx[sl] = c.vx;
      s.vy[sl] = c.vy;
      s.hasgoal8[sl] = static_cast<unsigned char>(c.hasgoal != 0);
      s.swp[sl] = c.sw;
      s.fcx[sl] = c.fx;
      s.fcy[sl] = c.fy;
      s.fjx[sl] = s.fjy[sl] = 0.0;
    }
  } else {
    const agent_consts c0 = load_agent_consts(late_args_of<BATCH>(Lb), F32);
    for (int sl = lane; sl < A; sl += WAVE) {
      const double px = L.agent_pos[2 * sl], py = L.agent_pos[2 * sl + 1];
      const double vx = L.agent_vel[2 * sl], vy = L.agent_vel[2 * sl + 1];
      const sfw_agent_const c = L.agent_c[sl];
      s.px[sl] = px;
      s.py[sl] = py;
      s.vx[sl] = vx;
      s.vy[sl] = vy;
      s.hasgoal8[sl] = static_cast<unsigned char>(c.has_goal != 0);
      s.swp[sl] = 0.0;
      double fx = 0.0, fy = 0.0;
      if (sl != 0) {
        desired_force(c0, px, py, vx, vy, c.has_goal != 0, c.goal_x, c.goal_y, c.goal_radius, c.desired_velocity, fx, fy);
        if (OBS && O > 0) {
          double tx, ty, sc;
          obstacle_sums<R>(k0, c0, obs_global(L.obstacles), px, py, c.radius, tx, ty, sc);
          fx = fma(tx, sc, fx);
          fy = fma(ty, sc, fy);
        }
      }
      if (L.agent_rest) {
        fx += L.agent_rest[2 * sl];
        fy += L.agent_rest[2 * sl + 1];
      }
      s.fcx[sl] = fx;
      s.fcy[sl] = fy;
      s.fjx[sl] = s.fjy[sl] = 0.0;
    }
  }
  if (OBS && O > 0) {
    const agent_consts c0 = load_agent_consts(late_args_of<BATCH>(Lb), F32);
    for (int sl = lane; sl < A; sl += WAVE) s.oscale[sl] = obstacle_scale<R>(k0, c0, L.agent_c[sl].radius);
  }
  for (int sl = A + lane; sl < cap; sl += WAVE) {
    s.px[sl] = s.py[sl] = s.vx[sl] = s.vy[sl] = 0.0;
    s.fcx[sl] = s.fcy[sl] = s.fjx[sl] = s.fjy[sl] = 0.0;
  }
  K2_SYNC();
  auto add_group_forces = [&](const sfm_consts<R> &k, const agent_consts &c) {
    for (int q = lane; q < NG; q += WAVE) s.gcen[q] = double2{0.0, 0.0};
    K2_SYNC();
    for (int sl = lane; sl < A; sl += WAVE)
      if (s.grp[sl] >= 0) {
        atomicAdd(&s.gcen[s.grp[sl]].x, s.px[sl]);
        atomicAdd(&s.gcen[s.grp[sl]].y, s.py[sl]);
      }
    K2_SYNC();
    for (int sl = lane; sl < A; sl += WAVE)
      if (sl != 0) {
        const double2 gf = group_force<R>(k, c, s, NG, 0, A, sl, sl, s.px[sl], s.py[sl]);
        s.fcx[sl] += gf.x;
        s.fcy[sl] += gf.y;
      }
    K2_SYNC();
  };
  if constexpr (GROUPS) {
    if (!L.resume) add_group_forces(k0, load_agent_consts(late_args_of<BATCH>(Lb), F32));
  }

  const int P = A * (A - 1) / 2;
  const int n_it = (P + WAVE - 1) / WAVE;
  const uint16_t *const tab_i = L.pair_tab, *const tab_j = L.pair_tab + static_cast<size_t>(n_it) * WAVE;
  const uint32_t lane_off = 2u * static_cast<uint32_t>(lane);

  const int64_t unit_vel_v = CYCLE ? 0 : L.rstep_stride + vel_row_of(L, rsample);
  const int64_t unit_pos = rsample,
                unit_vel = static_cast<int64_t>(
                    (static_cast<uint64_t>(static_cast<uint32_t>(__builtin_amdgcn_readfirstlane(static_cast<int>(unit_vel_v >> 32)))) << 32) |
                    static_cast<uint32_t>(__builtin_amdgcn_readfirstlane(static_cast<int>(unit_vel_v))));
  auto fetch_robot = [&](const sfw_unit *ptab, int64_t row_units, int st, int buf) {
    if constexpr (CYCLE) return;
    int l2 = lane;
    asm volatile("" : "+v"(l2));
    if (l2 < 2) {
      const char *src = reinterpret_cast<const char *>(ptab + static_cast<int64_t>(st) * row_units + (l2 ? unit_vel : unit_pos));
      __builtin_amdgcn_global_load_lds((const __attribute__((address_space(1))) void *)src,
                                       (__attribute__((address_space(3))) void *)(reinterpret_cast<char *>(s.rsb + buf)), 16,
                                       0, 0);
    }
  };
  if (step_begin < step_end) fetch_robot(L.ptab, L.row_units, step_begin, step_begin & 1);
  constexpr bool FIRST_IN_REGS = CAP == 64;
  uint32_t i0 = 0, j0 = 0;
  if constexpr (FIRST_IN_REGS) {
    if (n_it > 0) {
      load_pair_entries(tab_i, tab_j, lane_off, i0, j0);
      wait_pair_entries(i0, j0);
    }
  }

  auto pair_at = [&](const sfm_consts<R> &k, uint32_t io, uint32_t jo) {
    R qx, qy;
    if constexpr (CAP > 0) {
      double pix, piy, vix, viy, pjx, pjy, vjx, vjy;
      lds_pair_state<8 * CAP, 16 * CAP, 24 * CAP>(io, jo, pix, piy, vix, viy, pjx, pjy, vjx, vjy);
      pair_force_state<R>(k, pix, piy, vix, viy, pjx, pjy, vjx, vjy, qx, qy);
    } else {
      pair_force_state<R>(k, lds_at<double>(smem, io), lds_at<double>(smem, io + PY), lds_at<double>(smem, io + VX),
                          lds_at<double>(smem, io + VY), lds_at<double>(smem, jo), lds_at<double>(smem, jo + PY),
                          lds_at<double>(smem, jo + VX), lds_at<double>(smem, jo + VY), qx, qy);
    }
    atomicAdd(&lds_at<double>(smem, io + FCX), static_cast<double>(qx));
    atomicAdd(&lds_at<double>(smem, io + FCY), static_cast<double>(qy));
    atomicAdd(&lds_at<double>(smem, jo + FJX), static_cast<double>(qx));
    atomicAdd(&lds_at<double>(smem, jo + FJY), static_cast<double>(qy));
  };

  [[maybe_unused]] int cyc_ready = 0;
  for (int step = step_begin; step < step_end; ++step) {
    sfm_consts<R> k = k0;
    if constexpr (OBS) {
      k.pc.leading_here();
      k.lambda = sfwm::vgpr_copy_here(s_lambda);
      k.neg_l2e_inv_gamma = sfwm::vgpr_copy_here(s_nig);
      k.l2_f_social = sfwm::vgpr_copy_here(s_lfs);
      k.c_vel = sfwm::vgpr_copy_here(s_cvel);
      k.c_ang = sfwm::vgpr_copy_here(s_cang);
    }
    if constexpr (FIRST_IN_REGS) {
    if (n_it > 0) {
      uint32_t ia, ja, ib, jb;
      const uint16_t *ti = tab_i + WAVE, *tj = tab_j + WAVE;
      int left = n_it - 1;
      if (left >= 1) load_pair_entries(ti, tj, lane_off, ia, ja);
      pair_at(k, i0, j0);
      ti += WAVE;
      tj += WAVE;
      for (; left >= 2; left -= 2, ti += 2 * WAVE, tj += 2 * WAVE) {
        wait_pair_entries(ia, ja);
        load_pair_entries(ti, tj, lane_off, ib, jb);
        pair_at(k, ia, ja);
        wait_pair_entries(ib, jb);
        if (left > 2) load_pair_entries(ti + WAVE, tj + WAVE, lane_off, ia, ja);
        pair_at(k, ib, jb);
      }
      if (left == 1) {
        wait_pair_entries(ia, ja);
        pair_at(k, ia, ja);
      }
    }
    asm volatile("s_waitcnt vmcnt(0)" ::: "memory");
    } else {
    if (n_it > 0) {
      uint32_t ia, ja, ib, jb;
      load_pair_entries(tab_i, tab_j, lane_off, ia, ja);
      int left = n_it;
      const uint16_t *ti = tab_i + WAVE, *tj = tab_j + WAVE;
      for (; left >= 2; left -= 2, ti += 2 * WAVE, tj += 2 * WAVE) {
        wait_pair_entries(ia, ja);
        load_pair_entries(ti, tj, lane_off, ib, jb);
        pair_at(k, ia, ja);
        wait_pair_entries(ib, jb);
        if (left > 2) load_pair_entries(ti + WAVE, tj + WAVE, lane_off, ia, ja);
        pair_at(k, ib, jb);
      }
      if (left == 1) {
        wait_pair_entries(ia, ja);
        pair_at(k, ia, ja);
      }
    } else {
      asm volatile("s_waitcnt vmcnt(0)" ::: "memory");
    }
    }
    K2_SYNC();
    const late_launch La = late_args_of<BATCH>(Lb);
    const agent_consts c = load_agent_consts(La, F32);
    const sfw_agent_const *const agent_c = La->agent_c;
    if constexpr (CYCLE) {
      if (step >= cyc_ready) cyc_ready = cycle_wait_ready(res, step + 1);
    }
    const sfw_robot_step rs = CYCLE ? sfw_robot_step{k1->xs[step + 1], k1->ys[step + 1], k1->vxs[step], k1->vys[step]} : s.rsb[step & 1];
    if (step + 1 < step_end) fetch_robot(La->ptab, La->row_units, step + 1, (step + 1) & 1);
    const bool with_obs = OBS && c.O > 0;
    int lane_s = lane;
    asm volatile("" : "+v"(lane_s));
    for (int sl = lane_s; sl < A; sl += WAVE) {
      const agent_k ak = CONSTS_IN_LDS ? agent_k_lds(s, sl) : agent_k_global(agent_c, sl);
      double px = s.px[sl], py = s.py[sl], vx = s.vx[sl], vy = s.vy[sl];
      double nfx, nfy;
      int hg = s.hasgoal8[sl];
      const int hg0 = hg;
      bool contact;
      const double w = agent_step<R>(k, c, rs, ak, sl == 0, ak.id != c.robot_id, hg, contact, px, py, vx, vy,
                                     s.fcx[sl] - s.fjx[sl], s.fcy[sl] - s.fjy[sl], nfx, nfy);
      if (sl != 0 && hg0) s.hasgoal8[sl] = static_cast<unsigned char>(hg);
      if (contact) s.dead[0] = 2 + step;
      if (sl == 0 && with_obs) {
        s.wr[0] = w;
      } else {
        s.swp[sl] += w;
      }
      if (sl == 0) {
        px = rs.x;
        py = rs.y;
        vx = rs.vx;
        vy = rs.vy;
      }
      if constexpr (CAPTURE) {
        const size_t o = static_cast<size_t>(step) * static_cast<size_t>(A) + static_cast<size_t>(sl);
        double2 *const st = reinterpret_cast<double2 *>(cw.state) + 2 * o;
        st[0] = double2{px, py};
        st[1] = double2{vx, vy};
        double we = w;
        if (sl != 0 && ak.id != c.robot_id && w < wp_floor_of<R>::v) we = small_wp(k.pc, La, rs, px, py, vx, vy);
        if (!(sl == 0 && with_obs)) cw.work[o] = we;
        cw.has_goal[o] = sl == 0 ? 0 : hg;
      }
      if (!(sl == 0 && with_obs)) {
        s.px[sl] = px;
        s.py[sl] = py;
        s.vx[sl] = vx;
        s.vy[sl] = vy;
      }
      s.fcx[sl] = nfx;
      s.fcy[sl] = nfy;
      s.fjx[sl] = 0.0;
      s.fjy[sl] = 0.0;
    }
    if (with_obs) {
      K2_SYNC();
      if (c.obs_tasks) {
        const int Lseg = (c.O + OBS_SEG - 1) / OBS_SEG, seg = lane >> 2, sub = lane & (OBS_AGENT_LANES - 1);
        const R nis = sfwm::vgpr_const(static_cast<R>(-c.l2e_inv_sigma));
        const double2 *const pts_g = reinterpret_cast<const double2 *>(c.obstacles);
        const obs_lds_ptr pts_l = (obs_lds_ptr)s.obs;
        const bool in_lds = s.obs != nullptr;
        const double *const part = reinterpret_cast<const double *>(s.opart);
        constexpr int KA = OBS_AGENTS_PER_LANE;
        for (int a0 = 0; a0 < A; a0 += OBS_AGENT_LANES * KA) {
          const int nj = min(KA, (A - a0 + OBS_AGENT_LANES - 1) / OBS_AGENT_LANES);
          double pxj[KA], pyj[KA];
          R axj[KA + 1], ayj[KA + 1];
#pragma unroll
          for (int j = 0; j < KA; ++j) {
            pxj[j] = pyj[j] = 0.0;
            if (j < nj) {
              const int a = min(a0 + sub + OBS_AGENT_LANES * j, A - 1);
              pxj[j] = s.px[a];
              pyj[j] = s.py[a];
            }
          }
#pragma unroll
          for (int j = 0; j <= KA; ++j) axj[j] = ayj[j] = R(0);
          auto run_uniform = [&](auto pts) {
            switch (nj) {
              case 1: obstacle_segment_multi_uniform<R, 1>(k, pts, c.O, Lseg, seg, pxj, pyj, nis, axj, ayj); break;
              case 2: obstacle_segment_multi_uniform<R, 2>(k, pts, c.O, Lseg, seg, pxj, pyj, nis, axj, ayj); break;
              case (KA > 3 ? 3 : -1): obstacle_segment_multi_uniform<R, 3>(k, pts, c.O, Lseg, seg, pxj, pyj, nis, axj, ayj); break;
              default: obstacle_segment_multi_uniform<R, KA>(k, pts, c.O, Lseg, seg, pxj, pyj, nis, axj, ayj); break;
            }
          };
          if (in_lds) run_uniform(pts_l);
          else run_uniform(pts_g);
          auto reduce = [&](auto sl_tag) {
            constexpr int SL = decltype(sl_tag)::value;
            static_assert(KA <= 4 && (SL == 2 || KA % SL == 0), "OBS_AGENTS_PER_LANE: at most four agent slots per lane");
#pragma unroll
            for (int j0 = 0; j0 < KA; j0 += SL) {
              if (j0 < nj) {
#pragma unroll
                for (int u = 0; u < SL; ++u)
                  s.opart[u * WAVE + lane] = double2{static_cast<double>(axj[j0 + u]), static_cast<double>(ayj[j0 + u])};
                K2_SYNC();
                const int comp = lane & 1, js = (lane >> 1) & (SL - 1), gsub = lane / (2 * SL);
                const int a = a0 + gsub + OBS_AGENT_LANES * (j0 + js);
                if (lane < 8 * SL && a < A) {
                  const double *const col = part + 2 * (WAVE * js + gsub) + comp;
                  double v[OBS_SEG];
#pragma unroll
                  for (int q = 0; q < OBS_SEG; ++q) v[q] = col[2 * OBS_AGENT_LANES * q];
                  double *const acc = (comp == 0 ? s.fcx : s.fcy) + a;
                  const double sc = s.oscale[a], acc0 = *acc, wr0 = s.wr[0];
                  asm volatile("" ::: "memory");
// ... 12 lines not shown
                K2_SYNC();
              }
            }
          };
          if (in_lds && nj > 2) reduce(std::integral_constant<int, (KA >= 4 ? 4 : 2)>{});
          else reduce(std::integral_constant<int, 2>{});
        }
      } else {
        for (int a = lane; a < A; a += WAVE) {
          const double rad = CONSTS_IN_LDS ? s.ac[a].radius : agent_c[a].radius;
          double tx, ty, sc;
          obstacle_sums<R>(k, c, obs_global(c.obstacles), s.px[a], s.py[a], rad, tx, ty, sc);
          if (a == 0) {
            const double wr = s.wr[0] + fast_norm(tx * sc, ty * sc);
            s.swp[0] += wr;
            if constexpr (CAPTURE) cw.work[static_cast<size_t>(step) * static_cast<size_t>(A)] = wr;
          } else {
            s.fcx[a] = fma(tx, sc, s.fcx[a]);
            s.fcy[a] = fma(ty, sc, s.fcy[a]);
          }
        }
        K2_SYNC();
      }
      if (lane == 0) {
        s.px[0] = rs.x;
        s.py[0] = rs.y;
        s.vx[0] = rs.vx;
        s.vy[0] = rs.vy;
      }
    }
    if (const double *const pin = La->pin_rest) {
      if (pin_at_rest(pin, rs))
        for (int sl = lane_s; sl < A; sl += WAVE) {
          if (sl == 0) {
            s.fcx[0] += pin[2];
            s.fcy[0] += pin[3];
          } else {
            s.swp[sl] += pin[4 + sl];
            if constexpr (CAPTURE) cw.work[static_cast<size_t>(step) * static_cast<size_t>(A) + static_cast<size_t>(sl)] += pin[4 + sl];
          }
        }
    }
    K2_SYNC();
    if (s.dead[0] != 0) break;
    if constexpr (GROUPS) add_group_forces(k, c);
  }
  asm volatile("s_waitcnt vmcnt(0)" ::: "memory");
  const late_launch Le = late_args_of<BATCH>(Lb);
  if (Le->phase == SFW_PHASE_PREFIX) {
    sfw_cls_agent *rec = Le->out_state + first_local * A;
    for (int sl = lane; sl < A; sl += WAVE) {
      sfw_cls_agent c;
      c.px = s.px[sl]; c.py = s.py[sl]; c.vx = s.vx[sl]; c.vy = s.vy[sl];
      c.fx = s.fcx[sl]; c.fy = s.fcy[sl]; c.sw = s.swp[sl];
      c.hasgoal = s.hasgoal8[sl];
      c.pad = 0;
      rec[sl] = c;
    }
    if (lane == 0) Le->out_dead[first_local] = s.dead[0];
    if constexpr (!BATCH) clock_probe(1);
    return;
  }
  double sw_acc = 0.0;
  for (int sl = lane; sl < A; sl += WAVE) sw_acc += s.swp[sl];
  if constexpr (CYCLE) {
    for (int off = WAVE / 2; off > 0; off >>= 1) sw_acc += __shfl_down(sw_acc, off, WAVE);
    if (lane == 0) {
      res->social_work = sw_acc;
      res->dead = s.dead[0];
    }
  } else {
    finish_wave(s, lane, 1, 1, first_local, sw_acc);
  }
  if constexpr (!BATCH) clock_probe(1);
}
#undef K2_SYNC
template <typename R, bool GROUPS, int CAP, bool OBS>
__global__ void __launch_bounds__(WAVE, (GROUPS || CAP == 0) ? 1 : OBS ? SFW_FLAT_WAVES : SFW_FLAT_WAVES_NOOBS) sfw_social_kernel_flat(const sfw_launch L, const int G_unused) {
  sfwm::fp_mode_for_omod();
  extern __shared__ __attribute__((aligned(16))) char smem[];
  (void)G_unused;
  social_flat_wave<R, GROUPS, CAP, OBS, false>(L, smem, nullptr, nullptr, blockIdx.x, gridDim.x, L.item_base);
}
template <typename R, bool GROUPS>
__global__ void __launch_bounds__(WAVE, 1) sfw_crowd_kernel(const sfw_launch L, const sfw_crowd_out cw) {
  sfwm::fp_mode_for_omod();
  extern __shared__ __attribute__((aligned(16))) char smem[];
  social_flat_wave<R, GROUPS, 0, true, false, false, true>(L, smem, nullptr, nullptr, blockIdx.x, gridDim.x, 0, nullptr, cw);
}
template <typename R>
__global__ void __launch_bounds__(WAVE, 6) sfw_social_kernel_mixed(const sfw_launch L, const int G, const int n_reg, const int keep) {
  sfwm::fp_mode_for_omod();
  extern __shared__ __attribute__((aligned(16))) char smem[];
  if (blockIdx.x < static_cast<unsigned>(n_reg)) {
    sfw_launch Lr = L;
    if (Lr.phase == SFW_PHASE_PREFIX) Lr.n_cls = keep;
    else Lr.chunk_count = keep;
    social_reg_wave<R, 1, false>(Lr, G, smem, blockIdx.x, static_cast<unsigned>(n_reg));
  } else {
    social_flat_wave<R, false, 64, false, false>(L, smem, nullptr, nullptr, blockIdx.x - static_cast<unsigned>(n_reg),
                                                 gridDim.x - static_cast<unsigned>(n_reg), keep);
  }
}

__device__ __forceinline__ bool sel_less(const sfw_sel &a, const sfw_sel &b) {
  if (a.cost != b.cost) return a.cost < b.cost;
  if (a.neg_linvel != b.neg_linvel) return a.neg_linvel < b.neg_linvel;
  if (a.abs_angvel != b.abs_angvel) return a.abs_angvel < b.abs_angvel;
  return a.neg_index < b.neg_index;
}
__device__ __forceinline__ sfw_sel sel_empty() {
  sfw_sel e;
  e.cost = INFINITY;
  e.neg_linvel = INFINITY;
  e.abs_angvel = INFINITY;
  e.neg_index = 0x7fffffffffffffffLL;
  e.n_valid = 0;
  return e;
}
__device__ __forceinline__ sfw_sel sel_merge(const sfw_sel &a, const sfw_sel &b) {
  sfw_sel r = sel_less(b, a) ? b : a;
  r.n_valid = a.n_valid + b.n_valid;
  return r;
}
__device__ __forceinline__ sfw_sel sel_shfl_down(const sfw_sel &a, int off) {
  sfw_sel r;
  r.cost = __shfl_down(a.cost, off, WAVE);
  r.neg_linvel = __shfl_down(a.neg_linvel, off, WAVE);
  r.abs_angvel = __shfl_down(a.abs_angvel, off, WAVE);
  r.neg_index = __shfl_down(a.neg_index, off, WAVE);
  r.n_valid = __shfl_down(a.n_valid, off, WAVE);
  return r;
}
template <bool LIST = false>
__device__ __forceinline__ void sel_consider(sfw_sel &best, double c, const double *linvels, const double *angvels, int nw,
                                             int64_t t, int64_t index_base) {
  if (!(c >= 0.0)) return;
  best.n_valid += 1;
  const double lin = linvels[LIST ? t : t / nw], ang = angvels[LIST ? t : t % nw];
  const bool selectable = c < 10000.0 || (c == 10000.0 && (lin > 0.0 || (lin == 0.0 && ang == 0.0)));
  if (!selectable) return;
  sfw_sel cand;
  cand.cost = c;
  cand.neg_linvel = -lin;
  cand.abs_angvel = fabs(ang);
  cand.neg_index = -(index_base + t);
  cand.n_valid = 0;
  const long long nv = best.n_valid;
  if (sel_less(cand, best)) best = cand;
  best.n_valid = nv;
}
constexpr int ARGMIN_BLOCK = 256;
__device__ __forceinline__ sfw_sel block_reduce(sfw_sel v) {
  __shared__ sfw_sel wave_best[ARGMIN_BLOCK / WAVE];
  for (int off = WAVE / 2; off > 0; off >>= 1) v = sel_merge(v, sel_shfl_down(v, off));
  const int lane = threadIdx.x & (WAVE - 1), wid = threadIdx.x / WAVE;
  if (lane == 0) wave_best[wid] = v;
  __syncthreads();
  if (threadIdx.x == 0) {
    for (int w = 1; w < ARGMIN_BLOCK / WAVE; ++w) v = sel_merge(v, wave_best[w]);
  }
  return v;
}

template <bool LIST>
__global__ void __launch_bounds__(ARGMIN_BLOCK)
// ... 609 lines not shown
  typedef const __attribute__((address_space(4))) sfw_batch_rec *rec_ptr;
  const first_ptr f = (first_ptr)first;
  const unsigned b = blockIdx.x;
  int lo = 0, hi = B;
  while (hi - lo > 1) {
    const int mid = (lo + hi) >> 1;
    if (f[mid] <= b) lo = mid;
    else hi = mid;
  }
  const rec_ptr r = (rec_ptr)recs + lo;
  const late_launch Lb = (late_launch)&r->L;
  cycle_block<R, GROUPS, OBS, true, false>(*(const sfw_launch *)Lb, Lb, r->k2_bytes, b - f[lo], f[lo + 1] - f[lo]);
}

}



struct wave_plan { int G; int ns; bool flat; };
static wave_plan plan_for(int A, int64_t T, int O, int form, int cus) {
  if (A <= 0) return wave_plan{1, 1, false};
  const int P = A * (A - 1) / 2;
  const int rows = A / 2;
  const wave_plan flat{1, 0, true};
  const wave_plan reg = (A <= WAVE) ? wave_plan{WAVE / A < 32 ? WAVE / A : 32, 1, false} : wave_plan{1, 2, false};
  wave_plan best = flat;
  if (P == 0) {
    best = reg;
  } else if (A <= 2 * WAVE) {
    const double c_flat = 1.03 * (85.0 * ((P + WAVE - 1) / WAVE) + 215.0 * ((A + WAVE - 1) / WAVE));
    const double c_reg = (A <= WAVE) ? (90.0 * rows + 225.0) / reg.G : 0.9 * (180.0 * rows + 450.0);
    if (c_reg < c_flat) best = reg;
  }
  if (T <= static_cast<int64_t>(A <= 8 ? 6 : A <= 12 ? 12 : 16) * cus && (A >= 2 || O > 0)) best = flat;
  if (form == SFW_K2_FLAT && (A >= 2 || O > 0)) best = flat;
  if (form == SFW_K2_REGISTER && A <= 2 * WAVE) best = reg;
  return best;
}

int sfw_samples_per_wave(int A, int64_t T, int form, int cus) { return plan_for(A, T, 0, form, cus).G; }

int sfw_social_organisation(int A, int64_t T, int O, int form, int cus) {
  if (A <= 0) return SFW_ORG_NONE;
  const wave_plan pl = plan_for(A, T, O, form, cus);
  return pl.flat ? SFW_ORG_FLAT : pl.ns == 2 ? SFW_ORG_REGISTER_2 : SFW_ORG_REGISTER_1;
}

void sfw_derive(sfw_launch &L) {
  const sfw_params &p = L.p;
  sfw_force_k<double> &d = L.k.d;
  d.lambda = p.sfm_lambda;
  const double l2e = 1.4426950408889634074;
  d.neg_l2e_inv_gamma = -l2e / p.sfm_gamma;
  d.l2_f_social = std::log2(p.sfm_force_factor_social);
  d.c_vel = -(p.sfm_n_prime * p.sfm_n_prime) * (p.sfm_gamma * p.sfm_gamma) * l2e;
  d.c_ang = -(p.sfm_n * p.sfm_n) * (p.sfm_gamma * p.sfm_gamma) * l2e;
  d.l2_f_obstacle = p.sfm_force_factor_obstacle > 0 ? std::log2(p.sfm_force_factor_obstacle) : -1000.0;
  d.l2e_inv_sigma = l2e / p.sfm_force_sigma_obstacle;
  sfw_force_k<float> &f = L.k.f;
  f.lambda = static_cast<float>(d.lambda);
  f.neg_l2e_inv_gamma = static_cast<float>(d.neg_l2e_inv_gamma);
  f.l2_f_social = static_cast<float>(d.l2_f_social);
  f.c_vel = static_cast<float>(d.c_vel);
  f.c_ang = static_cast<float>(d.c_ang);
  f.l2_f_obstacle = static_cast<float>(d.l2_f_obstacle);
  f.l2e_inv_sigma = static_cast<float>(d.l2e_inv_sigma);
  L.k.f_desired = p.sfm_force_factor_desired;
  L.k.inv_tau = 1.0 / p.sfm_relaxation_time;
  L.k.rr = static_cast<double>(static_cast<float>(p.robot_radius) * static_cast<float>(p.robot_radius));
  L.k.inv_O = L.O > 0 ? 1.0 / L.O : 0.0;
  {
    const int A = L.A, O = L.O, Lseg = (O + OBS_SEG - 1) / OBS_SEG;
    const int full = A / (OBS_AGENT_LANES * OBS_AGENTS_PER_LANE), rest = (A % (OBS_AGENT_LANES * OBS_AGENTS_PER_LANE) + OBS_AGENT_LANES - 1) / OBS_AGENT_LANES;
    const double red = 40.0;
    const double c_tasks = full * (27.0 * Lseg * OBS_AGENTS_PER_LANE + 2 * red) + (rest ? 27.0 * Lseg * rest + ((rest + 1) / 2) * red : 0.0);
    const double c_lane = 27.0 * O * ((A + WAVE - 1) / WAVE);
    L.k.obs_tasks = (O > 0 && c_tasks < c_lane) ? 1 : 0;
  }
}

static int flat_cap(int A) { return A < 64 ? 64 : A < 104 ? 104 : A < 128 ? 128 : A < 208 ? 208 : A < 256 ? 256 : 0; }
static int flat_cap_runtime(int A) { return (A + 2) & ~1; }

static size_t lds_bytes_for(const wave_plan &pl, int A, int O, int NG, int n_grp_mem, bool obs_lds);
static bool obs_in_lds(const wave_plan &pl, int A, int O, int NG, int n_grp_mem, int64_t items, int cus) {
  return pl.flat && O > 0 && items <= static_cast<int64_t>(8) * cus && lds_bytes_for(pl, A, O, NG, n_grp_mem, true) <= 64 * 1024;
}
static size_t lds_bytes_for(const wave_plan &pl, int A, int O, int NG, int n_grp_mem, bool obs_lds) {
  if (pl.flat) {
    const int c = flat_cap(A);
    return lds_layout(nullptr, A, c > 0 ? c : flat_cap_runtime(A), A, 1, O, NG, n_grp_mem, NG > 0, true, obs_lds).bytes;
  }
  (void)obs_lds;
  return lds_layout(nullptr, A, WAVE * pl.ns, pl.G * A, pl.G, O, NG, n_grp_mem, true, false).bytes;
}

size_t sfw_social_lds_bytes(int A, int O, int NG, int n_grp_mem, int64_t T, int form, int cus) {
  const wave_plan pl = plan_for(A, T, O, form, cus);
  const size_t a = lds_bytes_for(pl, A, O, NG, n_grp_mem, obs_in_lds(pl, A, O, NG, n_grp_mem, T, cus));
  const wave_plan fl{1, 0, true};
  const size_t b = (A >= 2 || O > 0) ? lds_bytes_for(fl, A, O, NG, n_grp_mem, obs_in_lds(fl, A, O, NG, n_grp_mem, 1, cus)) : 0;
  return a > b ? a : b;
}

int64_t sfw_pair_table_entries(int A) {
  const int64_t P = static_cast<int64_t>(A) * (A - 1) / 2;
  const int64_t n = (P + WAVE - 1) / WAVE * WAVE;
  return 2 * (n > 0 ? n : WAVE);
}

hipError_t sfw_launch_pair_table(uint16_t *tab, int A, hipStream_t stream, bool runtime_cap) {
  const int n = static_cast<int>(sfw_pair_table_entries(A) / 2);
  const int cap = (!runtime_cap && flat_cap(A) > 0) ? flat_cap(A) : flat_cap_runtime(A);
  hipLaunchKernelGGL(sfw_pair_table_kernel, dim3((n + 255) / 256), dim3(256), 0, stream, tab, A, n, cap - A);
  return hipGetLastError();
}

static bool sfw_k1a_threads() {
  const char *e = std::getenv("SFW_K1A_THREADS");
  return e && e[0] == '1';
}

bool sfw_rollout_is_fused(const sfw_launch &L) { return L.chunk_count <= 2048 && L.S <= K1_SMALL_MAX_STEPS; }

hipError_t sfw_launch_rollout_poses(const sfw_launch &L, hipStream_t stream) {
  if (L.chunk_count <= 0) return hipSuccess;
  if (sfw_rollout_is_fused(L)) {
    hipLaunchKernelGGL((L.n_knots > 1 ? sfw_rollout_small_kernel<true, true> : L.list ? sfw_rollout_small_kernel<true> : sfw_rollout_small_kernel<false>),
                       dim3(static_cast<unsigned>(L.chunk_count)), dim3(K1_SMALL_BLOCK), 0, stream, L);
    return hipGetLastError();
  }
  const int block = 64;
  if (sfw_k1a_threads()) {
    const unsigned grid = static_cast<unsigned>((L.chunk_count + block - 1) / block);
    hipLaunchKernelGGL((L.n_knots > 1 ? sfw_rollout_kernel<true, true> : L.list ? sfw_rollout_kernel<true> : sfw_rollout_kernel<false>),
                       dim3(grid), dim3(block), 0, stream, L);
    return hipGetLastError();
  }
  constexpr int per_wave = WAVE / K1A_TEAM;
  const unsigned grid = static_cast<unsigned>((L.chunk_count + per_wave - 1) / per_wave);
  hipLaunchKernelGGL((L.n_knots > 1 ? sfw_rollout_team_kernel<true, true> : L.list ? sfw_rollout_team_kernel<true> : sfw_rollout_team_kernel<false>),
                     dim3(grid), dim3(block), 0, stream, L);
  return hipGetLastError();
}

hipError_t sfw_launch_rollout_costmap(const sfw_launch &L, hipStream_t stream) {
  if (L.chunk_count <= 0 || sfw_rollout_is_fused(L)) return hipSuccess;
  {
    const int block = 256;
    const int64_t n = L.chunk_count * L.S;
    const unsigned grid = static_cast<unsigned>((n + block - 1) / block);
    hipLaunchKernelGGL((L.list ? sfw_footprint_kernel<true> : sfw_footprint_kernel<false>), dim3(grid), dim3(block), 0, stream, L);
  }
  {
    const int block = 256;
    const unsigned grid = static_cast<unsigned>((L.chunk_count + block - 1) / block);
    hipLaunchKernelGGL(sfw_costmap_scan_kernel, dim3(grid), dim3(block), 0, stream, L);
  }
  return hipGetLastError();
}

hipError_t sfw_launch_rollout(const sfw_launch &L, hipStream_t stream) {
  hipError_t e = sfw_launch_rollout_poses(L, stream);
  return e != hipSuccess ? e : sfw_launch_rollout_costmap(L, stream);
}

template <typename K> static hipError_t launch_social_as(K kernel, const sfw_launch &L, int G, unsigned grid,
                                                          size_t lds, hipStream_t stream) {
  if (lds > 64 * 1024) {
    hipError_t e = hipFuncSetAttribute(reinterpret_cast<const void *>(kernel),
                                       hipFuncAttributeMaxDynamicSharedMemorySize, static_cast<int>(lds));
    if (e != hipSuccess) return e;
  }
  hipLaunchKernelGGL(kernel, dim3(grid), dim3(WAVE), lds, stream, L, G);
  return hipGetLastError();
}

template <int CAP> static bool reg_layout_matches() {
  const lds_layout s(nullptr, 5, CAP, 10, 2, 3, 0, 0, true, false);
  auto at = [&](const void *p) { return static_cast<int>(reinterpret_cast<const char *>(p) - reinterpret_cast<const char *>(s.px)); };
  using off = reg_off<CAP>;
  return at(s.py) == off::PY && at(s.vx) == off::VX && at(s.vy) == off::VY && at(s.fjx) == off::FJX && at(s.fjy) == off::FJY &&
         at(s.hasgoal) == off::HG && at(s.swp) == off::SW && at(s.dead) == off::DEAD && at(s.rsb) == off::RSB && s.hg_stride == 2;
}

static int64_t split_point(const wave_plan &pl, int A, int O, int NG, int form, int64_t items, int cus) {
  if (form != SFW_K2_AUTO || pl.flat || pl.ns != 1 || A < 2 || A > WAVE || NG > 0) return items;
  const int64_t S = 4LL * cus, W = (items + pl.G - 1) / pl.G, q = W / S;
  if (q < 1 || q > 5 || W % S == 0) return items;
  const int64_t reg_items = q * S * pl.G, rest = items - reg_items;
  const int P = A * (A - 1) / 2, Lseg = (O + OBS_SEG - 1) / OBS_SEG;
  const double c_reg_wave = 90.0 * (A / 2) + 225.0 + 24.0 * O;
  const double c_flat_wave = 1.03 * (85.0 * ((P + WAVE - 1) / WAVE) + 215.0) + 24.7 * ((A + OBS_AGENT_LANES - 1) / OBS_AGENT_LANES) * Lseg;
  const double t_now = static_cast<double>(q + 1), t_split = q + static_cast<double>((rest + S - 1) / S) * c_flat_wave / c_reg_wave;
  return t_split < 0.97 * t_now ? reg_items : items;
}

int64_t sfw_social_flat_items(int A, int O, int NG, int64_t T, int form, int cus) {
  if (A <= 0 || T <= 0) return 0;
  return T - split_point(plan_for(A, T, O, form, cus), A, O, NG, form, T, cus);
}

template <typename R> static hipError_t launch_social_typed(const sfw_launch &L_in, hipStream_t stream, const sfw_split_streams *sp = nullptr) {
  const int64_t all_items = L_in.phase == SFW_PHASE_PREFIX ? static_cast<int64_t>(L_in.n_cls) : L_in.chunk_count;
  const int64_t item_base = L_in.item_base, items = all_items - item_base;
  const int cus = L_in.n_cu > 0 ? L_in.n_cu : SFW_DEFAULT_CUS;
  const wave_plan pl = plan_for(L_in.A, items, L_in.O, L_in.k2_form, cus);
  if (sp && sp->side && item_base == 0) {
    const int64_t keep = L_in.pair_tab ? split_point(pl, L_in.A, L_in.O, L_in.NG, L_in.k2_form, items, cus) : items;
    if (keep < items && L_in.O == 0 && flat_cap(L_in.A) == 64) {
      const unsigned n_reg = static_cast<unsigned>((keep + pl.G - 1) / pl.G), n_flat = static_cast<unsigned>(items - keep);
      const wave_plan fl{1, 0, true};
      const size_t lds = std::max(lds_bytes_for(pl, L_in.A, 0, 0, 0, false), lds_bytes_for(fl, L_in.A, 0, 0, 0, false));
      sfw_launch L = L_in;
      L.k.obs_lds = 0;
      hipLaunchKernelGGL((sfw_social_kernel_mixed<R>), dim3(n_reg + n_flat), dim3(WAVE), lds, stream, L, pl.G, static_cast<int>(n_reg),
                         static_cast<int>(keep));
      return hipGetLastError();
    }
    if (keep < items) {
      sfw_launch La = L_in, Lb = L_in;
      if (La.phase == SFW_PHASE_PREFIX) La.n_cls = static_cast<int32_t>(keep);
      else La.chunk_count = keep;
      La.k2_form = SFW_K2_REGISTER;
      Lb.item_base = static_cast<int32_t>(keep);
      Lb.k2_form = SFW_K2_FLAT;
      Lb.clock_probe = nullptr;
      hipError_t e = hipEventRecord(sp->fork, stream);
      if (e == hipSuccess) e = hipStreamWaitEvent(sp->side, sp->fork, 0);
      if (e == hipSuccess) e = launch_social_typed<R>(La, stream);
      if (e == hipSuccess) e = launch_social_typed<R>(Lb, sp->side);
      if (e == hipSuccess) e = hipEventRecord(sp->join, sp->side);
      if (e == hipSuccess) e = hipStreamWaitEvent(stream, sp->join, 0);
      return e;
    }
  }
  const unsigned grid = static_cast<unsigned>((items + pl.G - 1) / pl.G);
  sfw_launch L = L_in;
  L.k.obs_lds = (item_base == 0 && obs_in_lds(pl, L.A, L.O, L.NG, L.n_grp_mem, items, cus)) ? 1 : 0;
  const size_t lds = lds_bytes_for(pl, L.A, L.O, L.NG, L.n_grp_mem, L.k.obs_lds != 0);
  if (lds > 160 * 1024) return hipErrorInvalidValue;
  static const bool layout_ok = reg_layout_matches<WAVE>() && reg_layout_matches<2 * WAVE>();
  if (!layout_ok) return hipErrorInvalidValue;
  const bool groups = L.NG > 0;
  if (!pl.flat && pl.G > lds_layout::REG_DEAD_CAP) return hipErrorInvalidValue;
  if (pl.flat) {
    if (8 * (static_cast<int64_t>(L.A) + 1) > 65535 || !L.pair_tab) return hipErrorInvalidValue;
    const bool obs = L.O > 0;
    switch (flat_cap(L.A)) {
      case 64:
        return groups ? launch_social_as(sfw_social_kernel_flat<R, true, 64, true>, L, 1, grid, lds, stream)
               : obs  ? launch_social_as(sfw_social_kernel_flat<R, false, 64, true>, L, 1, grid, lds, stream)
                      : launch_social_as(sfw_social_kernel_flat<R, false, 64, false>, L, 1, grid, lds, stream);
      case 104:
        return groups ? launch_social_as(sfw_social_kernel_flat<R, true, 104, true>, L, 1, grid, lds, stream)
               : obs  ? launch_social_as(sfw_social_kernel_flat<R, false, 104, true>, L, 1, grid, lds, stream)
                      : launch_social_as(sfw_social_kernel_flat<R, false, 104, false>, L, 1, grid, lds, stream);
      case 128:
        return groups ? launch_social_as(sfw_social_kernel_flat<R, true, 128, true>, L, 1, grid, lds, stream)
               : obs  ? launch_social_as(sfw_social_kernel_flat<R, false, 128, true>, L, 1, grid, lds, stream)
                      : launch_social_as(sfw_social_kernel_flat<R, false, 128, false>, L, 1, grid, lds, stream);
      case 208:
        return groups ? launch_social_as(sfw_social_kernel_flat<R, true, 208, true>, L, 1, grid, lds, stream)
               : obs  ? launch_social_as(sfw_social_kernel_flat<R, false, 208, true>, L, 1, grid, lds, stream)
                      : launch_social_as(sfw_social_kernel_flat<R, false, 208, false>, L, 1, grid, lds, stream);
      case 256:
        return groups ? launch_social_as(sfw_social_kernel_flat<R, true, 256, true>, L, 1, grid, lds, stream)
               : obs  ? launch_social_as(sfw_social_kernel_flat<R, false, 256, true>, L, 1, grid, lds, stream)
                      : launch_social_as(sfw_social_kernel_flat<R, false, 256, false>, L, 1, grid, lds, stream);
      default:
        return groups ? launch_social_as(sfw_social_kernel_flat<R, true, 0, true>, L, 1, grid, lds, stream)
               : obs  ? launch_social_as(sfw_social_kernel_flat<R, false, 0, true>, L, 1, grid, lds, stream)
                      : launch_social_as(sfw_social_kernel_flat<R, false, 0, false>, L, 1, grid, lds, stream);
    }
  }
  if (groups) {
    if (pl.ns == 1) return launch_social_as(sfw_social_kernel<R, 1, true>, L, pl.G, grid, lds, stream);
    return launch_social_as(sfw_social_kernel<R, 2, true>, L, pl.G, grid, lds, stream);
  }
  if (pl.ns == 1) return launch_social_as(sfw_social_kernel<R, 1, false>, L, pl.G, grid, lds, stream);
  return launch_social_as(sfw_social_kernel<R, 2, false>, L, pl.G, grid, lds, stream);
}

namespace {
__global__ void __launch_bounds__(256) sfw_no_social_kernel(const sfw_launch L) {
  const int64_t i = static_cast<int64_t>(blockIdx.x) * blockDim.x + threadIdx.x;
  if (i >= L.chunk_count) return;
  const int64_t t = L.chunk_begin + i;
  if (L.status[t] == SFW_ST_VALID) {
    L.costs[t] = sfw_cost_add_social(L.base_cost[t], L.p.social_weight, 0.0);
    sfw_put_term(L.terms, L.terms_T, t, SFW_TERM_SOCIAL, 0.0);
  }
}
}

hipError_t sfw_launch_social(const sfw_launch &L, hipStream_t stream, const sfw_split_streams *sp) {
  if (L.chunk_count <= 0 || L.A <= 0) return hipSuccess;
  if (L.A == 1 && L.O == 0 && L.NG == 0 && L.phase != SFW_PHASE_PREFIX && !L.out_state) {
    hipLaunchKernelGGL(sfw_no_social_kernel, dim3(static_cast<unsigned>((L.chunk_count + 255) / 256)), dim3(256), 0, stream, L);
    return hipGetLastError();
  }
#ifndef SFW_STRICT_BUILD
  if (L.p.precision == SFW_PRECISION_F32) return launch_social_typed<float>(L, stream, sp);
#endif
  return launch_social_typed<double>(L, stream, sp);
}

template <typename R> static hipError_t launch_crowd_typed(const sfw_launch &L_in, const sfw_crowd_out &cw, hipStream_t stream) {
  sfw_launch L = L_in;
  L.k.obs_lds = 0;
  L.item_base = 0;
  const bool groups = L.NG > 0;
  const size_t lds = lds_layout(nullptr, L.A, flat_cap_runtime(L.A), L.A, 1, L.O, L.NG, L.n_grp_mem, groups, true, false).bytes;
  if (lds > 160 * 1024 || 8 * (static_cast<int64_t>(L.A) + 1) > 65535 || !L.pair_tab) return hipErrorInvalidValue;
  if (L.chunk_count != 1 || L.phase != SFW_PHASE_WHOLE || L.resume || !cw.state || !cw.work || !cw.has_goal) return hipErrorInvalidValue;
  auto kernel = groups ? sfw_crowd_kernel<R, true> : sfw_crowd_kernel<R, false>;
  if (lds > 64 * 1024) {
    hipError_t e = hipFuncSetAttribute(reinterpret_cast<const void *>(kernel), hipFuncAttributeMaxDynamicSharedMemorySize,
                                       static_cast<int>(lds));
    if (e != hipSuccess) return e;
  }
  hipLaunchKernelGGL(kernel, dim3(1), dim3(WAVE), lds, stream, L, cw);
  return hipGetLastError();
}

hipError_t sfw_launch_crowd(const sfw_launch &L, const sfw_crowd_out &cw, hipStream_t stream) {
  if (L.A <= 0) return hipErrorInvalidValue;
#ifndef SFW_STRICT_BUILD
  if (L.p.precision == SFW_PRECISION_F32) return launch_crowd_typed<float>(L, cw, stream);
#endif
  return launch_crowd_typed<double>(L, cw, stream);
// ... 261 lines not shown
```

social_force_window_planner_amd/csrc/sfw_kernels_strict.hip:

```cpp
#define SFW_STRICT_BUILD 1
#define SFW_ASIN_DEG 8
#define SFW_EXP_DEG 9
#define sfw_launch_social sfw_launch_social_strict
#define sfw_launch_cycle sfw_launch_cycle_strict
#define sfw_launch_cycle_batch sfw_launch_cycle_batch_strict
#define sfw_launch_crowd sfw_launch_crowd_strict
#define sfw_cycle_batch_variant sfw_strict_unused_cycle_batch_variant
#define sfw_cycle_batch_record sfw_strict_unused_cycle_batch_record
#define sfw_cycle_applies sfw_strict_unused_cycle_applies
#define sfw_samples_per_wave sfw_strict_unused_samples_per_wave
#define sfw_social_organisation sfw_strict_unused_social_organisation
#define sfw_derive sfw_strict_unused_derive
#define sfw_social_flat_items sfw_strict_unused_social_flat_items
#define sfw_social_lds_bytes sfw_strict_unused_social_lds_bytes
#define sfw_pair_table_entries sfw_strict_unused_pair_table_entries
#define sfw_launch_pair_table sfw_strict_unused_launch_pair_table
#define sfw_rollout_is_fused sfw_strict_unused_rollout_is_fused
#define sfw_launch_rollout_poses sfw_strict_unused_launch_rollout_poses
#define sfw_launch_rollout_costmap sfw_strict_unused_launch_rollout_costmap
#define sfw_launch_rollout sfw_strict_unused_launch_rollout
#define sfw_launch_key_table sfw_strict_unused_launch_key_table
#define sfw_argmin_partials sfw_strict_unused_argmin_partials
#define sfw_launch_argmin sfw_strict_unused_launch_argmin
#define sfw_rescore_blocks sfw_strict_unused_rescore_blocks
#define sfw_launch_rescore sfw_strict_unused_launch_rescore
#define sfw_launch_ensemble sfw_strict_unused_launch_ensemble
#include "sfw_kernels.hip"
```

social_force_window_planner_amd/planner.py:

```python
from __future__ import annotations

import ctypes as C
import os
import subprocess

import numpy as np

from ._abi import (
    EXPORTED_SYMBOLS,
    SFW_ENSEMBLE_MAX,
    SFW_ENSEMBLE_MEAN,
    SFW_ERR_NO_DEVICE,
    SFW_OK,
    SfwAgent,
    SfwBatchDesc,
    SfwBest,
    SfwBestKey,
    SfwBlendStat,
    SFW_BLEND_MAX_L,
    SfwGoalArgs,
    SfwMppi,
    SFW_MPPI_MAX_ITER,
    SfwParams,
    SfwPerturb,
    SfwRobotState,
    SfwPlanInfo,
    SfwWeights,
    SFW_N_TERMS,
    default_params,
)

_HERE = os.path.dirname(os.path.abspath(__file__))
LIB_PATH = os.environ.get("SFW_HIP_LIB") or os.path.join(_HERE, "libsfw_hip.so")
_lib = None


class SfwError(RuntimeError):
    def __init__(self, status, what, detail=""):
        super().__init__(f"{what} failed: status {status}" + (f" ({detail})" if detail else ""))
        self.status = status


def build(force=False):
    csrc = os.path.join(_HERE, "csrc")
    srcs = [os.path.join(csrc, f) for f in ("sfw_capi.hip", "sfw_kernels.hip", "sfw_kernels_strict.hip", "sfw_device.h", "sfw_math.h")]
    srcs.append(os.path.join(_HERE, "..", "include", "sfw_hip.h"))
    stale = (not os.path.exists(LIB_PATH)) or any(
        os.path.getmtime(LIB_PATH) < os.path.getmtime(s) for s in srcs)
    if force or stale:
        r = subprocess.run(["make", "-C", csrc, "all"], capture_output=True, text=True)
        if r.returncode != 0:
            raise RuntimeError("building libsfw_hip.so failed:\n" + r.stdout + r.stderr)
    return LIB_PATH


def lib():
    global _lib
    if _lib is None:
        if not os.path.exists(LIB_PATH):
            raise FileNotFoundError(
                f"{LIB_PATH} is missing: run `python -c 'import __graft_entry__ as g; g.build()'` "
                "(there is no CPU fallback for the scoring path)")
        L = C.CDLL(LIB_PATH)
        vp = C.c_void_p
        L.sfw_params_default.argtypes = [C.POINTER(SfwParams)]
        L.sfw_params_default.restype = None
        L.sfw_abi_version.restype = C.c_int
        L.sfw_create.argtypes = [C.POINTER(SfwParams), C.c_int, C.POINTER(vp)]
        L.sfw_destroy.argtypes = [vp]
        L.sfw_set_params.argtypes = [vp, C.POINTER(SfwParams)]
        L.sfw_last_error.argtypes = [vp]
        L.sfw_last_error.restype = C.c_char_p
        L.sfw_set_costmap.argtypes = [vp, vp, C.c_uint32, C.c_uint32, C.c_double, C.c_double, C.c_double]
        L.sfw_set_footprint.argtypes = [vp, vp, C.c_int32]
        L.sfw_set_agents.argtypes = [vp, vp, C.c_int32, vp, C.c_int32]
        L.sfw_score_grid.argtypes = [vp, C.POINTER(SfwRobotState), vp, C.c_int32, vp, C.c_int32,
                                     C.POINTER(SfwGoalArgs), vp, C.POINTER(SfwBest)]
        L.sfw_score_one.argtypes = [vp, C.POINTER(SfwRobotState), C.c_double, C.c_double, C.c_double,
                                    C.POINTER(SfwGoalArgs), C.POINTER(C.c_double), vp, C.c_int32,
                                    C.POINTER(C.c_int32)]
        L.sfw_grid_stage.argtypes = [vp, C.POINTER(SfwRobotState), vp, C.c_int32, vp, C.c_int32,
                                     C.POINTER(SfwGoalArgs), C.c_int64]
        L.sfw_grid_launch.argtypes = [vp]
        L.sfw_grid_sync.argtypes = [vp]
        L.sfw_grid_fetch.argtypes = [vp, vp, C.POINTER(SfwBest), C.POINTER(SfwBestKey)]
        L.sfw_grid_plan_info.argtypes = [vp, C.POINTER(SfwPlanInfo)]
        L.sfw_set_k2_form.argtypes = [vp, C.c_int32]
        L.sfw_set_timing.argtypes = [vp, C.c_int32]
        L.sfw_last_launch_ms.argtypes = [vp, C.c_int32, C.POINTER(C.c_float)]
        L.sfw_last_clock_ghz.argtypes = [vp, C.POINTER(C.c_double)]
        L.sfw_grid_points.argtypes = [vp, C.c_int64, vp, C.c_int32, C.POINTER(C.c_int32)]
        L.sfw_grid_points_batch.argtypes = [vp, C.c_int64, C.c_int64, vp, vp]
        L.sfw_set_points_capture.argtypes = [vp, C.c_int32]
        L.sfw_stream.argtypes = [vp]
        L.sfw_stream.restype = vp
        L.sfw_multi_create.argtypes = [C.POINTER(SfwParams), C.POINTER(C.c_int), C.c_int32, C.c_int32, C.POINTER(vp)]
        L.sfw_multi_destroy.argtypes = [vp]
        L.sfw_multi_last_error.argtypes = [vp]
        L.sfw_multi_last_error.restype = C.c_char_p
        L.sfw_multi_ranks.argtypes = [vp]
        L.sfw_multi_ranks.restype = C.c_int32
        L.sfw_multi_rank_handle.argtypes = [vp, C.c_int32]
        L.sfw_multi_rank_handle.restype = vp
        L.sfw_multi_set_params.argtypes = [vp, C.POINTER(SfwParams)]
        L.sfw_multi_set_costmap.argtypes = [vp, vp, C.c_uint32, C.c_uint32, C.c_double, C.c_double, C.c_double]
        L.sfw_multi_set_footprint.argtypes = [vp, vp, C.c_int32]
        L.sfw_multi_set_agents.argtypes = [vp, vp, C.c_int32, vp, C.c_int32]
        L.sfw_multi_score_grid.argtypes = [vp, C.POINTER(SfwRobotState), vp, C.c_int32, vp, C.c_int32,
                                           C.POINTER(SfwGoalArgs), vp, C.POINTER(SfwBest)]
        L.sfw_multi_last_us.argtypes = [vp, C.c_int32, C.POINTER(C.c_double)]
        L.sfw_multi_rank_rows.argtypes = [vp, C.c_int32, C.POINTER(C.c_int32), C.POINTER(C.c_int32)]
        L.sfw_plan_row_blocks.argtypes = [vp, C.c_int32, vp, C.c_int32, C.c_double, C.c_double, C.c_double, C.c_double,
                                          C.c_double, C.c_int32, C.c_int32, C.c_int32, vp]
        L.sfw_grid_costs_view.argtypes = [vp]
        L.sfw_grid_costs_view.restype = C.c_void_p
        L.sfw_plan_shared_prefix.argtypes = [vp, C.c_int32, vp, C.c_int32, C.c_double, C.c_double, C.c_double, C.c_double,
                                             C.c_double, C.c_int32, C.c_int32, vp, vp, C.c_int32, C.POINTER(C.c_int32)]
        L.sfw_multi_grid_points.argtypes = [vp, C.c_int64, vp, C.c_int32, C.POINTER(C.c_int32)]
        L.sfw_batch_create.argtypes = [C.POINTER(SfwParams), C.c_int, C.c_int32, C.POINTER(vp)]
        L.sfw_batch_destroy.argtypes = [vp]
        L.sfw_batch_last_error.argtypes = [vp]
        L.sfw_batch_last_error.restype = C.c_char_p
        L.sfw_batch_size.argtypes = [vp]
        L.sfw_batch_size.restype = C.c_int32
        L.sfw_batch_member.argtypes = [vp, C.c_int32]
        L.sfw_batch_member.restype = vp
        L.sfw_batch_launch.argtypes = [vp]
        L.sfw_batch_fetch.argtypes = [vp, vp]
        L.sfw_batch_score_grid.argtypes = [vp, vp, vp, C.c_int32, vp, C.c_int32, vp, vp]
        L.sfw_batch_describe.argtypes = [vp, C.POINTER(SfwBatchDesc)]
        L.sfw_batch_last_us.argtypes = [vp, C.c_int32, C.POINTER(C.c_double)]
        L.sfw_set_terms_capture.argtypes = [vp, C.c_int32]
        L.sfw_grid_rescore.argtypes = [vp, C.POINTER(SfwWeights), C.c_int32, C.POINTER(SfwBest), vp]
        L.sfw_grid_terms.argtypes = [vp, C.c_int64, C.c_int64, vp]
        L.sfw_ensemble_create.argtypes = [C.POINTER(SfwParams), C.c_int, C.c_int32, C.POINTER(vp)]
        L.sfw_ensemble_destroy.argtypes = [vp]
        L.sfw_ensemble_last_error.argtypes = [vp]
        L.sfw_ensemble_last_error.restype = C.c_char_p
        L.sfw_ensemble_size.argtypes = [vp]
        L.sfw_ensemble_size.restype = C.c_int32
        L.sfw_ensemble_member.argtypes = [vp, C.c_int32]
        L.sfw_ensemble_member.restype = vp
        L.sfw_ensemble_set_params.argtypes = [vp, C.POINTER(SfwParams)]
        L.sfw_ensemble_set_costmap.argtypes = [vp, vp, C.c_uint32, C.c_uint32, C.c_double, C.c_double, C.c_double]
        L.sfw_ensemble_set_footprint.argtypes = [vp, vp, C.c_int32]
        L.sfw_ensemble_set_hypothesis.argtypes = [vp, C.c_int32, vp, C.c_int32, vp, C.c_int32]
        L.sfw_ensemble_score_grid.argtypes = [vp, C.POINTER(SfwRobotState), vp, C.c_int32, vp, C.c_int32,
                                              C.POINTER(SfwGoalArgs), C.c_int32, vp, vp, vp, C.POINTER(SfwBest)]
        L.sfw_ensemble_aggregate.argtypes = [vp, C.c_int32, vp, vp, vp, C.POINTER(SfwBest)]
        L.sfw_ensemble_last_us.argtypes = [vp, C.c_int32, C.POINTER(C.c_double)]
        L.sfw_samples_stage.argtypes = [vp, C.POINTER(SfwRobotState), vp, vp, vp, C.c_int32, C.POINTER(SfwGoalArgs), C.c_int64]
        L.sfw_score_samples.argtypes = [vp, C.POINTER(SfwRobotState), vp, vp, vp, C.c_int32, C.POINTER(SfwGoalArgs), vp,
                                        C.POINTER(SfwBest)]
        L.sfw_score_one_crowd.argtypes = [vp, C.POINTER(SfwRobotState), C.c_double, C.c_double, C.c_double,
                                          C.POINTER(SfwGoalArgs), C.POINTER(C.c_double), vp, vp, vp, C.c_int32, C.c_int32,
                                          C.POINTER(C.c_int32)]
        L.sfw_grid_crowd.argtypes = [vp, C.c_int64, C.POINTER(C.c_double), vp, vp, vp, C.c_int32, C.c_int32,
                                     C.POINTER(C.c_int32)]
        L.sfw_sequences_stage.argtypes = [vp, C.POINTER(SfwRobotState), vp, vp, vp, C.c_int32, C.c_int32, vp,
                                          C.POINTER(SfwGoalArgs), C.c_int64]
        L.sfw_score_sequences.argtypes = [vp, C.POINTER(SfwRobotState), vp, vp, vp, C.c_int32, C.c_int32, vp,
                                          C.POINTER(SfwGoalArgs), vp, C.POINTER(SfwBest)]
        L.sfw_grid_blend.argtypes = [vp, vp, C.c_int32, vp, C.POINTER(SfwBlendStat), vp, vp]
        L.sfw_sequences_perturb_stage.argtypes = [vp, C.POINTER(SfwRobotState), C.POINTER(SfwPerturb), C.c_int32, C.c_int32, vp,
                                                  C.POINTER(SfwGoalArgs), C.c_int64]
        L.sfw_score_perturbed.argtypes = [vp, C.POINTER(SfwRobotState), C.POINTER(SfwPerturb), C.c_int32, C.c_int32, vp,
                                          C.POINTER(SfwGoalArgs), vp, C.POINTER(SfwBest)]
        L.sfw_sequences_knots.argtypes = [vp, C.c_int64, C.c_int64, vp, vp, vp]
        L.sfw_sequences_normals.argtypes = [vp, C.c_int64, C.c_int64, vp]
# ... 188 lines not shown

    @staticmethod
    def _perturb(seed, nominal, sigma, lo, hi, knot_steps, flags):
        nom = np.ascontiguousarray(_f64(nominal))
        ks = np.ascontiguousarray(np.asarray(knot_steps, dtype=np.int32).reshape(-1))
        if nom.ndim != 2 or nom.shape[1] != 3 or len(ks) != nom.shape[0]:
            raise ValueError("perturbed: nominal must be a (K, 3) array and knot_steps must hold K steps")
        p = SfwPerturb()
        p.seed = int(seed)
        p.nominal = nom.ctypes.data if nom.size else None
        for name, v in (("sigma", sigma), ("lo", lo), ("hi", hi)):
            setattr(p, name, (C.c_double * 3)(*[float(x) for x in np.asarray(v, dtype=np.float64).reshape(3)]))
        p.flags = int(flags)
        return p, nom, ks

    def stage_perturbed(self, robot_state, n, seed, nominal, sigma, lo, hi, knot_steps, goal_args, flags=0, index_base=0):
        p, nom, ks = self._perturb(seed, nominal, sigma, lo, hi, knot_steps, flags)
        rs, ga = SfwRobotState(*robot_state), SfwGoalArgs(*goal_args)
        K = nom.shape[0]
        self._check(lib().sfw_sequences_perturb_stage(self._h, C.byref(rs), C.byref(p), n, K, ks.ctypes.data if len(ks) else None,
                                                      C.byref(ga), index_base), "sfw_sequences_perturb_stage")
        self._mark_staged((n, 1), knots=K)

    def score_perturbed(self, robot_state, n, seed, nominal, sigma, lo, hi, knot_steps, goal_args, flags=0):
        p, nom, ks = self._perturb(seed, nominal, sigma, lo, hi, knot_steps, flags)
        rs, ga = SfwRobotState(*robot_state), SfwGoalArgs(*goal_args)
        K = nom.shape[0]
        costs = np.empty(max(n, 0), dtype=np.float64)
        best = SfwBest()
        self._check(lib().sfw_score_perturbed(self._h, C.byref(rs), C.byref(p), n, K, ks.ctypes.data if len(ks) else None,
                                              C.byref(ga), costs.ctypes.data if n > 0 else None, C.byref(best)), "sfw_score_perturbed")
        self._mark_staged((n, 1), knots=K)
        return costs, best.as_dict()

    def knots(self, first, count):
        K = getattr(self, "_n_knots", 1) if self._grid is not None else 1
        out = np.zeros((3, K, max(count, 1)), dtype=np.float64)
        self._check(lib().sfw_sequences_knots(self._h, first, count, out[0].ctypes.data, out[1].ctypes.data, out[2].ctypes.data),
                    "sfw_sequences_knots")
        return np.ascontiguousarray(out.transpose(1, 0, 2))

    def normals(self, first, count):
        K = getattr(self, "_n_knots", 1) if self._grid is not None else 1
        out = np.zeros((K, 3, max(count, 1)), dtype=np.float64)
        self._check(lib().sfw_sequences_normals(self._h, first, count, out.ctypes.data), "sfw_sequences_normals")
        return out

    def prepared(self, robot_state, linvels, angvels, goal_args, index_base=0, zero_copy=False):
        return PreparedGrid(self, robot_state, linvels, angvels, goal_args, index_base, zero_copy)

    def launch(self):
        self._check(lib().sfw_grid_launch(self._h), "sfw_grid_launch")

    def sync(self):
        self._check(lib().sfw_grid_sync(self._h), "sfw_grid_sync")

    def fetch(self, want_costs=True, out=None):
        nv, nw = self._grid
        if want_costs and out is not None:
            if out.dtype != np.float64 or out.size != nv * nw or not out.flags.c_contiguous:
                raise ValueError("fetch(out=...): need a contiguous float64 array of nv * nw elements")
            costs = out
        else:
            costs = np.empty(nv * nw, dtype=np.float64) if want_costs else None
        best, key = SfwBest(), SfwBestKey()
        self._check(lib().sfw_grid_fetch(self._h, costs.ctypes.data if want_costs else None, C.byref(best),
                                         C.byref(key)), "sfw_grid_fetch")
        return costs, best.as_dict(), key.as_tuple()

    def costs_view(self):
        p = lib().sfw_grid_costs_view(self._h)
        if not p:
            return None
        nv, nw = self._grid
        a = np.ctypeslib.as_array(C.cast(p, C.POINTER(C.c_double)), shape=(nv * nw,))
        a.flags.writeable = False
        return a

    def plan_info(self):
        info = SfwPlanInfo()
        self._check(lib().sfw_grid_plan_info(self._h, C.byref(info)), "sfw_grid_plan_info")
        return info.as_dict()

    def set_k2_form(self, form):
        self._check(lib().sfw_set_k2_form(self._h, form), "sfw_set_k2_form")

    def set_timing(self, enabled=True):
        self._check(lib().sfw_set_timing(self._h, 1 if enabled else 0), "sfw_set_timing")

    def last_launch_ms(self, which=0):
        ms = C.c_float()
        self._check(lib().sfw_last_launch_ms(self._h, which, C.byref(ms)), "sfw_last_launch_ms")
        return ms.value

    def sustained_clock_ghz(self):
        v = C.c_double()
        self._check(lib().sfw_last_clock_ghz(self._h, C.byref(v)), "sfw_last_clock_ghz")
        return v.value

    def set_points_capture(self, enabled=True):
        self._check(lib().sfw_set_points_capture(self._h, 1 if enabled else 0), "sfw_set_points_capture")

    def grid_points_batch(self, first, count, n_steps):
        pts = np.zeros((count, n_steps, 3), dtype=np.float64)
        n = np.zeros(count, dtype=np.int32)
        self._check(lib().sfw_grid_points_batch(self._h, first, count, pts.ctypes.data, n.ctypes.data),
                    "sfw_grid_points_batch")
        return pts, n

    def grid_points(self, index, points_cap=4096):
        pts = np.zeros((points_cap, 3), dtype=np.float64)
        n = C.c_int32()
        self._check(lib().sfw_grid_points(self._h, index, pts.ctypes.data, points_cap, C.byref(n)),
                    "sfw_grid_points")
        return pts[: min(n.value, points_cap)].copy()

    def _num_steps(self):
        n = int(self.params.sim_time / self.params.sim_granularity + 0.5)
        return n if n != 0 else 1

    @staticmethod
    def _crowd_buffers(cap, A):
        n = max(cap, 1) * max(A, 1)
        return (np.zeros(4 * n, dtype=np.float64)[: 4 * max(cap, 1) * A].reshape(max(cap, 1), A, 4),
                np.zeros(n, dtype=np.float64)[: max(cap, 1) * A].reshape(max(cap, 1), A),
                np.zeros(n, dtype=np.int32)[: max(cap, 1) * A].reshape(max(cap, 1), A))

    @staticmethod
    def _crowd_dict(cost, n, state, work, has_goal):
        m = min(n, state.shape[0])
        return {"cost": cost, "n_steps": n, "state": state[:m].copy(), "work": work[:m].copy(), "has_goal": has_goal[:m].copy()}

    def score_one_crowd(self, robot_state, vx_samp, vy_samp, vth_samp, goal_args, steps_cap=None):
        rs, ga = SfwRobotState(*robot_state), SfwGoalArgs(*goal_args)
        A, cap = self._n_agents, steps_cap if steps_cap is not None else self._num_steps()
        state, work, hg = self._crowd_buffers(cap, A)
        cost, n = C.c_double(), C.c_int32()
        self._check(lib().sfw_score_one_crowd(self._h, C.byref(rs), vx_samp, vy_samp, vth_samp, C.byref(ga), C.byref(cost),
                                              state.ctypes.data, work.ctypes.data, hg.ctypes.data, A, cap, C.byref(n)),
                    "sfw_score_one_crowd")
        self._grid = None
        return self._crowd_dict(cost.value, n.value, state, work, hg)

    def grid_crowd(self, index, steps_cap=None):
        A, cap = self._n_staged_agents, steps_cap if steps_cap is not None else self._num_steps()
        state, work, hg = self._crowd_buffers(cap, A)
        cost, n = C.c_double(), C.c_int32()
        self._check(lib().sfw_grid_crowd(self._h, index, C.byref(cost), state.ctypes.data, work.ctypes.data, hg.ctypes.data,
                                         A, cap, C.byref(n)), "sfw_grid_crowd")
        return self._crowd_dict(cost.value, n.value, state, work, hg)

    def set_terms_capture(self, enabled=True):
        self._check(lib().sfw_set_terms_capture(self._h, 1 if enabled else 0), "sfw_set_terms_capture")

    def cost_terms(self, first=0, count=None):
        if count is None:
            nv, nw = self._grid if self._grid is not None else (0, 0)
            count = max(nv * nw - first, 0)
        out = np.empty((count, SFW_N_TERMS), dtype=np.float64)
        self._check(lib().sfw_grid_terms(self._h, first, count, out.ctypes.data), "sfw_grid_terms")
        return out

    def rescore(self, weights, want_costs=False):
        w = np.ascontiguousarray(np.asarray(weights, dtype=np.float64).reshape(-1, SFW_N_TERMS))
        K = w.shape[0]
        best = (SfwBest * max(K, 1))()
# ... 506 lines not shown
```

Before: 7.593 million.

## Reuse pair-pass robot interaction terms for Wp cost instead of recomputing

The flat social kernel gets a variant in which the pair-force pass records the ev/ea interaction terms for robot-agent pairs into a new LDS plane. The next step's agent update then reads those terms to accumulate the social work cost Wp, rather than recomputing the robot-agent force separately. The pair table gains a per-wave ballot mask that marks robot lanes. The variant is enabled only when the extra LDS does not reduce waves per CU, with no groups and no pinned rest. The cost is more LDS, extra stores inside the hot pair loop, and a one-step-lagged accumulation path that has to stay numerically equivalent.

```diff
diff --git a/include/sfw_hip.h b/include/sfw_hip.h
--- a/include/sfw_hip.h
+++ b/include/sfw_hip.h
@@ -175,6 +175,7 @@
   int64_t rest_noise_unreproduced;
 } sfw_plan_info;
 int sfw_grid_plan_info(sfw_handle h, sfw_plan_info *out);
+int sfw_grid_wp_from_pairs(sfw_handle h, int32_t *on);
 int sfw_plan_shared_prefix(const double *linvels, int32_t nv,
                            const double *angvels, int32_t nw, double vx0,
                            double vtheta0, double acc_x, double acc_theta,
diff --git a/social_force_window_planner_amd/_abi.py b/social_force_window_planner_amd/_abi.py
--- a/social_force_window_planner_amd/_abi.py
+++ b/social_force_window_planner_amd/_abi.py
@@ -157,6 +157,7 @@
     "sfw_grid_fetch",
     "sfw_grid_costs_view",
     "sfw_grid_plan_info",
+    "sfw_grid_wp_from_pairs",
     "sfw_plan_shared_prefix",
     "sfw_plan_row_blocks",
     "sfw_plan_axis_classes",
diff --git a/social_force_window_planner_amd/csrc/sfw_capi.hip b/social_force_window_planner_amd/csrc/sfw_capi.hip
--- a/social_force_window_planner_amd/csrc/sfw_capi.hip
+++ b/social_force_window_planner_amd/csrc/sfw_capi.hip
@@ -114,6 +114,7 @@
     int n_cu = SFW_DEFAULT_CUS, n_xcd = SFW_DEFAULT_CUS / SFW_CUS_PER_XCD;
     std::vector<int> prefix_env;
     bool pin_rest_on = true;
+    bool wp_from_pairs_on = true;
     long spin_us = 20000;
     bool arena_direct_on = true;
     size_t mirror_max_bytes = size_t(64) << 20;
@@ -393,6 +394,7 @@
   sfw_derive(L);
   if (h->cfg.obs_tasks_force >= 0 && L.O > 0) L.k.obs_tasks = h->cfg.obs_tasks_force;
   L.pair_tab = h->pair_tab.p;
+  L.wp_from_pairs = h->cfg.wp_from_pairs_on ? 1 : 0;
   L.status = h->status.p;
   L.base_cost = h->base_cost.p;
   L.costs = h->costs.p;
@@ -1780,6 +1782,7 @@
   }
   if (const char *b = std::getenv("SFW_FORCE_FLAT")) h->live.k2_form = std::atoi(b) == 1 ? SFW_K2_FLAT : std::atoi(b) == 0 ? SFW_K2_REGISTER : SFW_K2_AUTO;
   if (const char *b = std::getenv("SFW_PIN_REST")) h->cfg.pin_rest_on = std::atoi(b) != 0;
+  if (const char *b = std::getenv("SFW_WP_FROM_PAIRS")) h->cfg.wp_from_pairs_on = std::atoi(b) != 0;
   if (const char *b = std::getenv("SFW_SPIN_US")) h->cfg.spin_us = std::max(0L, std::atol(b));
   if (const char *b = std::getenv("SFW_ARENA_DIRECT")) h->cfg.arena_direct_on = std::atoi(b) != 0;
   if (const char *b = std::getenv("SFW_MIRROR_MAX_MB")) h->cfg.mirror_max_bytes = static_cast<size_t>(std::max(0L, std::atol(b))) << 20;
@@ -2353,6 +2356,19 @@
   return SFW_OK;
 }
 
+int sfw_grid_wp_from_pairs(sfw_handle h, int32_t *on) {
+  if (!h || !on) return SFW_ERR_INVALID_ARG;
+  if (!h->st.valid) return fail(h, SFW_ERR_STATE, "grid_wp_from_pairs before grid_stage");
+  sfw_plan_info pi;
+  if (const int rc = sfw_grid_plan_info(h, &pi)) return rc;
+  const int64_t T = static_cast<int64_t>(h->st.nv) * h->st.nw, items = pi.chunks > 0 ? (T + pi.chunks - 1) / pi.chunks : T;
+  *on = (h->cfg.wp_from_pairs_on && !h->st.d_pin_rest && !pi.one_launch &&
+         sfw_social_wp_from_pairs(h->st.A, h->st.O, h->st.NG, h->st.n_grp_mem, items, h->live.k2_form, h->cfg.n_cu,
+                                  h->live.params.precision == SFW_PRECISION_F32))
+            ? 1 : 0;
+  return SFW_OK;
+}
+
 int sfw_set_k2_form(sfw_handle h, int32_t form) {
   if (!h) return SFW_ERR_INVALID_ARG;
   if (form != SFW_K2_AUTO && form != SFW_K2_REGISTER && form != SFW_K2_FLAT)
diff --git a/social_force_window_planner_amd/csrc/sfw_device.h b/social_force_window_planner_amd/csrc/sfw_device.h
--- a/social_force_window_planner_amd/csrc/sfw_device.h
+++ b/social_force_window_planner_amd/csrc/sfw_device.h
@@ -146,6 +146,7 @@
   int32_t n_knots;
   const int32_t *knot_step;
   int64_t knot_stride;
+  int32_t wp_from_pairs;
 };
 
 __device__ __forceinline__ void sfw_put_term(double *terms, int64_t T, int64_t t, int k, double v) {
@@ -257,6 +258,7 @@
 hipError_t sfw_launch_control_cost(const sfw_perturb_dev &a, const double *plan, int K, int64_t n, int64_t index_base,
                                    const double *z_kept, double gamma, const double *bias_add, double *bias, hipStream_t stream);
 hipError_t sfw_launch_key_table(const sfw_sel *sel, double *table, int r, int R, hipStream_t stream);
+bool sfw_social_wp_from_pairs(int A, int O, int NG, int n_grp_mem, int64_t items, int form, int cus, bool f32);
 int64_t sfw_pair_table_entries(int A);
 hipError_t sfw_launch_pair_table(uint16_t *tab, int A, hipStream_t stream, bool runtime_cap = false);
 int sfw_samples_per_wave(int A, int64_t T, int form, int cus);
diff --git a/social_force_window_planner_amd/csrc/sfw_kernels.hip b/social_force_window_planner_amd/csrc/sfw_kernels.hip
--- a/social_force_window_planner_amd/csrc/sfw_kernels.hip
+++ b/social_force_window_planner_amd/csrc/sfw_kernels.hip
@@ -712,9 +712,21 @@
   return __builtin_copysignf(mag, static_cast<float>(sgn));
 }
 
+template <typename R> __device__ __forceinline__ R pair_norm(R ev, R ea) {
+  const R q = fma(ev, ev, ea * ea);
+  R rq, nq;
+  sfwm::rsqrt_sqrt(fma(R(1), q, tiny_of<R>::v), rq, nq);
+  return q * rq;
+}
+
+__device__ __forceinline__ double add_unfused(double a, double b) {
+#pragma clang fp contract(off)
+  return a + b;
+}
+
 template <typename R, bool NORM_ONLY = false>
 __device__ __forceinline__ void pair_force(const sfm_consts<R> &k, R dx, R dy, R wx, R wy, double cw, R &fx,
-                                           R &fy) {
+                                           R &fy, R &ev_out, R &ea_out) {
   using namespace sfwm;
   const R tiny = tiny_of<R>::v;
   R rd, dn, rl, il;
@@ -732,25 +744,39 @@
   R ev, ea;
   exp2_fast2_gated(k.pc, fma(k.c_vel, t2, a), fma(k.c_ang, t2, a), cw, ev, ea);
   if constexpr (NORM_ONLY) {
-    const R q = fma(ev, ev, ea * ea);
-    R rq, nq;
-    rsqrt_sqrt(fma(R(1), q, tiny), rq, nq);
-    fx = q * rq;
+    ev_out = ev;
+    ea_out = ea;
+    fx = pair_norm(ev, ea);
     fy = R(0);
     return;
   }
   ea = copysign_from(ea, cw);
+  ev_out = ev;
+  ea_out = ea;
   const R gx = ix * rl, gy = iy * rl;
   fx = fma(ea, gy, -(ev * gx));
   fy = fma(-ev, gy, -(ea * gx));
+}
+template <typename R, bool NORM_ONLY = false>
+__device__ __forceinline__ void pair_force(const sfm_consts<R> &k, R dx, R dy, R wx, R wy, double cw, R &fx,
+                                           R &fy) {
+  R ev, ea;
+  pair_force<R, NORM_ONLY>(k, dx, dy, wx, wy, cw, fx, fy, ev, ea);
+}
+template <typename R, bool NORM_ONLY = false>
+__device__ __forceinline__ void pair_force_state(const sfm_consts<R> &k, double pix, double piy, double vix,
+                                                 double viy, double pjx, double pjy, double vjx, double vjy,
+                                                 R &fx, R &fy, R &ev, R &ea) {
+  const double dx = pjx - pix, dy = pjy - piy, wx = vix - vjx, wy = viy - vjy;
+  const double cw = fma(wx, dy, -(wy * dx));
+  pair_force<R, NORM_ONLY>(k, R(dx), R(dy), R(wx), R(wy), cw, fx, fy, ev, ea);
 }
 template <typename R, bool NORM_ONLY = false>
 __device__ __forceinline__ void pair_force_state(const sfm_consts<R> &k, double pix, double piy, double vix,
                                                  double viy, double pjx, double pjy, double vjx, double vjy,
                                                  R &fx, R &fy) {
-  const double dx = pjx - pix, dy = pjy - piy, wx = vix - vjx, wy = viy - vjy;
-  const double cw = fma(wx, dy, -(wy * dx));
-  pair_force<R, NORM_ONLY>(k, R(dx), R(dy), R(wx), R(wy), cw, fx, fy);
+  R ev, ea;
+  pair_force_state<R, NORM_ONLY>(k, pix, piy, vix, viy, pjx, pjy, vjx, vjy, fx, fy, ev, ea);
 }
 
 __device__ __forceinline__ double fast_norm(double x, double y) {
@@ -926,11 +952,12 @@
   double *oscale;
   int *hasgoal, *dead, *grp, *goff, *gmem;
   unsigned char *hasgoal8;
+  char *wcap;
   int hg_stride;
   size_t bytes;
   static constexpr int REG_DEAD_CAP = 32;
   __host__ __device__ lds_layout(char *base, int A, int cap, int GA, int G, int O, int NG, int NM, bool consts,
-                                 bool with_frc, bool obs_in_lds = false) {
+                                 bool with_frc, bool obs_in_lds = false, int wcap_elem = 0) {
     char *const base0 = base;
     auto take = [&](size_t n) {
       char *p = base;
@@ -976,6 +1003,7 @@
     grp = reinterpret_cast<int *>(take(sizeof(int) * (NG > 0 ? A : 0)));
     goff = reinterpret_cast<int *>(take(sizeof(int) * (NG > 0 ? NG + 1 : 0)));
     gmem = reinterpret_cast<int *>(take(sizeof(int) * (NG > 0 && NM > 0 ? NM : 0)));
+    wcap = take(with_frc ? 2 * static_cast<size_t>(wcap_elem) * static_cast<size_t>(cap) : 0);
     bytes = static_cast<size_t>(base - base0);
   }
   __device__ __forceinline__ int hg(int sl) const { return hg_stride == 1 ? static_cast<int>(hasgoal8[sl]) : hasgoal[sl * hg_stride]; }
@@ -1562,6 +1590,8 @@
   }
   tab[u] = static_cast<uint16_t>(8 * i);
   tab[n_entries + u] = static_cast<uint16_t>(8 * j);
+  const unsigned long long robot_lanes = __ballot(u < P && (i == 0 || j == 0));
+  if ((u & (WAVE - 1)) == 0) reinterpret_cast<unsigned long long *>(tab + 2 * static_cast<size_t>(n_entries))[u / WAVE] = robot_lanes;
 }
 
 __device__ __forceinline__ void load_pair_entries(const uint16_t *ti, const uint16_t *tj, uint32_t lane_off, uint32_t &io,
@@ -1600,12 +1630,13 @@
   return r;
 }
 #define K2_SYNC() do { if constexpr (CYCLE) wave_sync(); else __syncthreads(); } while (0)
-template <typename R, bool GROUPS, int CAP, bool OBS, bool CYCLE, bool BATCH = false, bool CAPTURE = false>
+template <typename R, bool GROUPS, int CAP, bool OBS, bool CYCLE, bool BATCH = false, bool CAPTURE = false, bool WP_PAIRS = false>
 __device__ __forceinline__ void social_flat_wave(const sfw_launch &L, char *const smem, const k1s_lds *const k1, cycle_result *const res,
                                                  const unsigned bid, const unsigned nblk, const int64_t item_base,
                                                  const late_launch Lb = nullptr, const sfw_crowd_out cw = sfw_crowd_out{}) {
   static_assert(CYCLE || !BATCH, "a batched wave is a cycle kernel's wave");
   static_assert(!CAPTURE || (!CYCLE && !BATCH), "the crowd capture runs as a kernel of its own");
+  static_assert(!WP_PAIRS || (!CYCLE && !CAPTURE && !GROUPS && CAP > 0), "Wp from the pair pass: a flat-form kernel of its own");
   const int lane = threadIdx.x;
   const int A = L.A, O = L.O;
   const int NG = GROUPS ? L.NG : 0;
@@ -1615,7 +1646,12 @@
   (void)FCX;
   (void)FCY;
   constexpr bool CONSTS_IN_LDS = GROUPS || CYCLE;
-  const lds_layout s(smem, A, cap, A, 1, O, NG, GROUPS ? L.n_grp_mem : 0, CONSTS_IN_LDS, true, L.k.obs_lds != 0);
+  const lds_layout s(smem, A, cap, A, 1, O, NG, GROUPS ? L.n_grp_mem : 0, CONSTS_IN_LDS, true, L.k.obs_lds != 0,
+                     WP_PAIRS ? static_cast<int>(sizeof(R)) : 0);
+  const int wcap_off = WP_PAIRS ? __builtin_amdgcn_readfirstlane(static_cast<int>(s.wcap - smem)) : 0;
+  const int WEA = 8 * cap;
+  (void)wcap_off;
+  (void)WEA;
   const int64_t first_local = CYCLE ? static_cast<int64_t>(bid) : item_base + xcd_contiguous(bid, nblk, static_cast<unsigned>(L.n_xcd));
   const sfm_consts<R> k0 = make_consts<R, true>(L);
   const sfw_force_k<R> &fk = force_k<R>(L);
@@ -1719,6 +1755,7 @@
   const int n_it = (P + WAVE - 1) / WAVE;
   const uint16_t *const tab_i = L.pair_tab, *const tab_j = L.pair_tab + static_cast<size_t>(n_it) * WAVE;
   const uint32_t lane_off = 2u * static_cast<uint32_t>(lane);
+  typedef const __attribute__((address_space(4))) unsigned long long *lane_masks;
 
   const int64_t unit_vel_v = CYCLE ? 0 : L.rstep_stride + vel_row_of(L, rsample);
   const int64_t unit_pos = rsample,
@@ -1737,7 +1774,7 @@
     }
   };
   if (step_begin < step_end) fetch_robot(L.ptab, L.row_units, step_begin, step_begin & 1);
-  constexpr bool FIRST_IN_REGS = CAP == 64;
+  constexpr bool FIRST_IN_REGS = CAP == 64 && !WP_PAIRS;
   uint32_t i0 = 0, j0 = 0;
   if constexpr (FIRST_IN_REGS) {
     if (n_it > 0) {
@@ -1746,21 +1783,41 @@
     }
   }
 
-  auto pair_at = [&](const sfm_consts<R> &k, uint32_t io, uint32_t jo) {
-    R qx, qy;
+  auto pair_at = [&](const sfm_consts<R> &k, uint32_t io, uint32_t jo, [[maybe_unused]] unsigned long long robot_lanes) {
+    R qx, qy, ev, ea;
     if constexpr (CAP > 0) {
       double pix, piy, vix, viy, pjx, pjy, vjx, vjy;
       lds_pair_state<8 * CAP, 16 * CAP, 24 * CAP>(io, jo, pix, piy, vix, viy, pjx, pjy, vjx, vjy);
-      pair_force_state<R>(k, pix, piy, vix, viy, pjx, pjy, vjx, vjy, qx, qy);
+      pair_force_state<R>(k, pix, piy, vix, viy, pjx, pjy, vjx, vjy, qx, qy, ev, ea);
     } else {
       pair_force_state<R>(k, lds_at<double>(smem, io), lds_at<double>(smem, io + PY), lds_at<double>(smem, io + VX),
                           lds_at<double>(smem, io + VY), lds_at<double>(smem, jo), lds_at<double>(smem, jo + PY),
-                          lds_at<double>(smem, jo + VX), lds_at<double>(smem, jo + VY), qx, qy);
+                          lds_at<double>(smem, jo + VX), lds_at<double>(smem, jo + VY), qx, qy, ev, ea);
+    }
+    if constexpr (WP_PAIRS) {
+      if (__builtin_amdgcn_inverse_ballot_w64(robot_lanes)) {
+        const uint32_t other = io + jo + static_cast<uint32_t>(wcap_off);
+        if constexpr (F32) {
+          lds_at<float2>(smem, other) = float2{static_cast<float>(ev), static_cast<float>(ea)};
+        } else {
+          lds_at<double>(smem, other) = static_cast<double>(ev);
+          lds_at<double>(smem, other + WEA) = static_cast<double>(ea);
+        }
+      }
     }
     atomicAdd(&lds_at<double>(smem, io + FCX), static_cast<double>(qx));
     atomicAdd(&lds_at<double>(smem, io + FCY), static_cast<double>(qy));
     atomicAdd(&lds_at<double>(smem, jo + FJX), static_cast<double>(qx));
     atomicAdd(&lds_at<double>(smem, jo + FJY), static_cast<double>(qy));
+  };
+
+  auto robot_lanes_of = [&](int it) -> unsigned long long {
+    if constexpr (WP_PAIRS) {
+      const uint16_t *const m = tab_j + (n_it * WAVE + 4 * it);
+      return *(lane_masks)(const __attribute__((address_space(1))) unsigned long long *)m;
+    } else {
+      return 0ull;
+    }
   };
 
   [[maybe_unused]] int cyc_ready = 0;
@@ -1780,20 +1837,20 @@
       const uint16_t *ti = tab_i + WAVE, *tj = tab_j + WAVE;
       int left = n_it - 1;
       if (left >= 1) load_pair_entries(ti, tj, lane_off, ia, ja);
-      pair_at(k, i0, j0);
+      pair_at(k, i0, j0, robot_lanes_of(0));
       ti += WAVE;
       tj += WAVE;
       for (; left >= 2; left -= 2, ti += 2 * WAVE, tj += 2 * WAVE) {
         wait_pair_entries(ia, ja);
         load_pair_entries(ti, tj, lane_off, ib, jb);
-        pair_at(k, ia, ja);
+        pair_at(k, ia, ja, robot_lanes_of(n_it - left));
         wait_pair_entries(ib, jb);
         if (left > 2) load_pair_entries(ti + WAVE, tj + WAVE, lane_off, ia, ja);
-        pair_at(k, ib, jb);
+        pair_at(k, ib, jb, robot_lanes_of(n_it - left + 1));
       }
       if (left == 1) {
         wait_pair_entries(ia, ja);
-        pair_at(k, ia, ja);
+        pair_at(k, ia, ja, robot_lanes_of(n_it - 1));
       }
     }
     asm volatile("s_waitcnt vmcnt(0)" ::: "memory");
@@ -1806,14 +1863,14 @@
       for (; left >= 2; left -= 2, ti += 2 * WAVE, tj += 2 * WAVE) {
         wait_pair_entries(ia, ja);
         load_pair_entries(ti, tj, lane_off, ib, jb);
-        pair_at(k, ia, ja);
+        pair_at(k, ia, ja, robot_lanes_of(n_it - left));
         wait_pair_entries(ib, jb);
         if (left > 2) load_pair_entries(ti + WAVE, tj + WAVE, lane_off, ia, ja);
-        pair_at(k, ib, jb);
+        pair_at(k, ib, jb, robot_lanes_of(n_it - left + 1));
       }
       if (left == 1) {
         wait_pair_entries(ia, ja);
-        pair_at(k, ia, ja);
+        pair_at(k, ia, ja, robot_lanes_of(n_it - 1));
       }
     } else {
       asm volatile("s_waitcnt vmcnt(0)" ::: "memory");
@@ -1831,6 +1888,7 @@
     const bool with_obs = OBS && c.O > 0;
     int lane_s = lane;
     asm volatile("" : "+v"(lane_s));
+    const bool wp_prev = WP_PAIRS && step > step_begin, wp_now = !WP_PAIRS || step + 1 == step_end;
     for (int sl = lane_s; sl < A; sl += WAVE) {
       const agent_k ak = CONSTS_IN_LDS ? agent_k_lds(s, sl) : agent_k_global(agent_c, sl);
       double px = s.px[sl], py = s.py[sl], vx = s.vx[sl], vy = s.vy[sl];
@@ -1838,14 +1896,31 @@
       int hg = s.hasgoal8[sl];
       const int hg0 = hg;
       bool contact;
-      const double w = agent_step<R>(k, c, rs, ak, sl == 0, ak.id != c.robot_id, hg, contact, px, py, vx, vy,
+      const bool wp_on = ak.id != c.robot_id;
+      const double w = agent_step<R>(k, c, rs, ak, sl == 0, wp_on && wp_now, hg, contact, px, py, vx, vy,
                                      s.fcx[sl] - s.fjx[sl], s.fcy[sl] - s.fjy[sl], nfx, nfy);
       if (sl != 0 && hg0) s.hasgoal8[sl] = static_cast<unsigned char>(hg);
       if (contact) s.dead[0] = 2 + step;
       if (sl == 0 && with_obs) {
         s.wr[0] = w;
       } else {
-        s.swp[sl] += w;
+        double sw = s.swp[sl];
+        if constexpr (WP_PAIRS) {
+          if (wp_prev && sl != 0 && wp_on) {
+            const unsigned o = 8u * static_cast<unsigned>(sl) + static_cast<unsigned>(wcap_off);
+            R ev, ea;
+            if constexpr (F32) {
+              const float2 e = lds_at<float2>(smem, o);
+              ev = e.x;
+              ea = e.y;
+            } else {
+              ev = lds_at<double>(smem, o);
+              ea = lds_at<double>(smem, o + WEA);
+            }
+            sw = add_unfused(sw, static_cast<double>(pair_norm<R>(ev, ea)));
+          }
+        }
+        s.swp[sl] = sw + w;
       }
       if (sl == 0) {
         px = rs.x;
@@ -2024,6 +2099,13 @@
   (void)G_unused;
   social_flat_wave<R, GROUPS, CAP, OBS, false>(L, smem, nullptr, nullptr, blockIdx.x, gridDim.x, L.item_base);
 }
+template <typename R, int CAP, bool OBS>
+__global__ void __launch_bounds__(WAVE, OBS ? SFW_FLAT_WAVES : SFW_FLAT_WAVES_NOOBS) sfw_social_kernel_flat_wp(const sfw_launch L, const int G_unused) {
+  sfwm::fp_mode_for_omod();
+  extern __shared__ __attribute__((aligned(16))) char smem[];
+  (void)G_unused;
+  social_flat_wave<R, false, CAP, OBS, false, false, false, true>(L, smem, nullptr, nullptr, blockIdx.x, gridDim.x, L.item_base);
+}
 template <typename R, bool GROUPS>
 __global__ void __launch_bounds__(WAVE, 1) sfw_crowd_kernel(const sfw_launch L, const sfw_crowd_out cw) {
   sfwm::fp_mode_for_omod();
@@ -2799,17 +2881,31 @@
 static int flat_cap(int A) { return A < 64 ? 64 : A < 104 ? 104 : A < 128 ? 128 : A < 208 ? 208 : A < 256 ? 256 : 0; }
 static int flat_cap_runtime(int A) { return (A + 2) & ~1; }
 
-static size_t lds_bytes_for(const wave_plan &pl, int A, int O, int NG, int n_grp_mem, bool obs_lds);
+static size_t lds_bytes_for(const wave_plan &pl, int A, int O, int NG, int n_grp_mem, bool obs_lds, int wcap_elem = 0);
 static bool obs_in_lds(const wave_plan &pl, int A, int O, int NG, int n_grp_mem, int64_t items, int cus) {
   return pl.flat && O > 0 && items <= static_cast<int64_t>(8) * cus && lds_bytes_for(pl, A, O, NG, n_grp_mem, true) <= 64 * 1024;
 }
-static size_t lds_bytes_for(const wave_plan &pl, int A, int O, int NG, int n_grp_mem, bool obs_lds) {
+static size_t lds_bytes_for(const wave_plan &pl, int A, int O, int NG, int n_grp_mem, bool obs_lds, int wcap_elem) {
   if (pl.flat) {
     const int c = flat_cap(A);
-    return lds_layout(nullptr, A, c > 0 ? c : flat_cap_runtime(A), A, 1, O, NG, n_grp_mem, NG > 0, true, obs_lds).bytes;
+    return lds_layout(nullptr, A, c > 0 ? c : flat_cap_runtime(A), A, 1, O, NG, n_grp_mem, NG > 0, true, obs_lds, wcap_elem).bytes;
   }
   (void)obs_lds;
   return lds_layout(nullptr, A, WAVE * pl.ns, pl.G * A, pl.G, O, NG, n_grp_mem, true, false).bytes;
+}
+
+static int flat_waves_per_cu(size_t lds, int O) {
+  const size_t granule = 1280, alloc = (lds + granule - 1) / granule * granule;
+  const int by_lds = alloc > 0 ? static_cast<int>(160 * 1024 / alloc) : 32;
+  const int by_regs = 4 * (O > 0 ? SFW_FLAT_WAVES : SFW_FLAT_WAVES_NOOBS);
+  return by_lds < by_regs ? by_lds : by_regs;
+}
+static bool wp_plane_is_free(const wave_plan &fl, int A, int O, int NG, int n_grp_mem, bool obs_lds, bool f32, int64_t items, int cus) {
+  if (A < 2 || NG > 0 || flat_cap(A) == 0) return false;
+  const size_t without = lds_bytes_for(fl, A, O, NG, n_grp_mem, obs_lds), with = lds_bytes_for(fl, A, O, NG, n_grp_mem, obs_lds, f32 ? 4 : 8);
+  const int64_t wanted = (items + cus - 1) / cus;
+  const int64_t w0 = std::min<int64_t>(wanted, flat_waves_per_cu(without, O)), w1 = std::min<int64_t>(wanted, flat_waves_per_cu(with, O));
+  return with <= 160 * 1024 && w1 == w0;
 }
 
 size_t sfw_social_lds_bytes(int A, int O, int NG, int n_grp_mem, int64_t T, int form, int cus) {
@@ -2823,11 +2919,12 @@
 int64_t sfw_pair_table_entries(int A) {
   const int64_t P = static_cast<int64_t>(A) * (A - 1) / 2;
   const int64_t n = (P + WAVE - 1) / WAVE * WAVE;
-  return 2 * (n > 0 ? n : WAVE);
+  const int64_t m = n > 0 ? n : WAVE;
+  return 2 * m + 4 * (m / WAVE);
 }
 
 hipError_t sfw_launch_pair_table(uint16_t *tab, int A, hipStream_t stream, bool runtime_cap) {
-  const int n = static_cast<int>(sfw_pair_table_entries(A) / 2);
+  const int n = static_cast<int>(sfw_pair_table_entries(A) * WAVE / (2 * WAVE + 4));
   const int cap = (!runtime_cap && flat_cap(A) > 0) ? flat_cap(A) : flat_cap_runtime(A);
   hipLaunchKernelGGL(sfw_pair_table_kernel, dim3((n + 255) / 256), dim3(256), 0, stream, tab, A, n, cap - A);
   return hipGetLastError();
@@ -2911,6 +3008,12 @@
   const double c_flat_wave = 1.03 * (85.0 * ((P + WAVE - 1) / WAVE) + 215.0) + 24.7 * ((A + OBS_AGENT_LANES - 1) / OBS_AGENT_LANES) * Lseg;
   const double t_now = static_cast<double>(q + 1), t_split = q + static_cast<double>((rest + S - 1) / S) * c_flat_wave / c_reg_wave;
   return t_split < 0.97 * t_now ? reg_items : items;
+}
+
+bool sfw_social_wp_from_pairs(int A, int O, int NG, int n_grp_mem, int64_t items, int form, int cus, bool f32) {
+  if (A <= 0 || items <= 0) return false;
+  const wave_plan pl = plan_for(A, items, O, form, cus);
+  return pl.flat && wp_plane_is_free(pl, A, O, NG, n_grp_mem, obs_in_lds(pl, A, O, NG, n_grp_mem, items, cus), f32, items, cus);
 }
 
 int64_t sfw_social_flat_items(int A, int O, int NG, int64_t T, int form, int cus) {
@@ -2931,6 +3034,7 @@
       const size_t lds = std::max(lds_bytes_for(pl, L_in.A, 0, 0, 0, false), lds_bytes_for(fl, L_in.A, 0, 0, 0, false));
       sfw_launch L = L_in;
       L.k.obs_lds = 0;
+      L.wp_from_pairs = 0;
       hipLaunchKernelGGL((sfw_social_kernel_mixed<R>), dim3(n_reg + n_flat), dim3(WAVE), lds, stream, L, pl.G, static_cast<int>(n_reg),
                          static_cast<int>(keep));
       return hipGetLastError();
@@ -2955,7 +3059,9 @@
   const unsigned grid = static_cast<unsigned>((items + pl.G - 1) / pl.G);
   sfw_launch L = L_in;
   L.k.obs_lds = (item_base == 0 && obs_in_lds(pl, L.A, L.O, L.NG, L.n_grp_mem, items, cus)) ? 1 : 0;
-  const size_t lds = lds_bytes_for(pl, L.A, L.O, L.NG, L.n_grp_mem, L.k.obs_lds != 0);
+  L.wp_from_pairs = (pl.flat && L_in.wp_from_pairs && !L.pin_rest && L.step_end - L.step_begin >= 2 &&
+                     wp_plane_is_free(pl, L.A, L.O, L.NG, L.n_grp_mem, L.k.obs_lds != 0, sizeof(R) == 4, items, cus)) ? 1 : 0;
+  const size_t lds = lds_bytes_for(pl, L.A, L.O, L.NG, L.n_grp_mem, L.k.obs_lds != 0, L.wp_from_pairs ? static_cast<int>(sizeof(R)) : 0);
   if (lds > 160 * 1024) return hipErrorInvalidValue;
   static const bool layout_ok = reg_layout_matches<WAVE>() && reg_layout_matches<2 * WAVE>();
   if (!layout_ok) return hipErrorInvalidValue;
@@ -2964,6 +3070,26 @@
   if (pl.flat) {
     if (8 * (static_cast<int64_t>(L.A) + 1) > 65535 || !L.pair_tab) return hipErrorInvalidValue;
     const bool obs = L.O > 0;
+    if (L.wp_from_pairs) {
+      switch (flat_cap(L.A)) {
+        case 64:
+          return obs ? launch_social_as(sfw_social_kernel_flat_wp<R, 64, true>, L, 1, grid, lds, stream)
+                     : launch_social_as(sfw_social_kernel_flat_wp<R, 64, false>, L, 1, grid, lds, stream);
+        case 104:
+          return obs ? launch_social_as(sfw_social_kernel_flat_wp<R, 104, true>, L, 1, grid, lds, stream)
+                     : launch_social_as(sfw_social_kernel_flat_wp<R, 104, false>, L, 1, grid, lds, stream);
+        case 128:
+          return obs ? launch_social_as(sfw_social_kernel_flat_wp<R, 128, true>, L, 1, grid, lds, stream)
+                     : launch_social_as(sfw_social_kernel_flat_wp<R, 128, false>, L, 1, grid, lds, stream);
+        case 208:
+          return obs ? launch_social_as(sfw_social_kernel_flat_wp<R, 208, true>, L, 1, grid, lds, stream)
+                     : launch_social_as(sfw_social_kernel_flat_wp<R, 208, false>, L, 1, grid, lds, stream);
+        case 256:
+          return obs ? launch_social_as(sfw_social_kernel_flat_wp<R, 256, true>, L, 1, grid, lds, stream)
+                     : launch_social_as(sfw_social_kernel_flat_wp<R, 256, false>, L, 1, grid, lds, stream);
+        default: return hipErrorInvalidValue;
+      }
+    }
     switch (flat_cap(L.A)) {
       case 64:
         return groups ? launch_social_as(sfw_social_kernel_flat<R, true, 64, true>, L, 1, grid, lds, stream)
diff --git a/social_force_window_planner_amd/csrc/sfw_kernels_strict.hip b/social_force_window_planner_amd/csrc/sfw_kernels_strict.hip
--- a/social_force_window_planner_amd/csrc/sfw_kernels_strict.hip
+++ b/social_force_window_planner_amd/csrc/sfw_kernels_strict.hip
@@ -12,6 +12,7 @@
 #define sfw_social_organisation sfw_strict_unused_social_organisation
 #define sfw_derive sfw_strict_unused_derive
 #define sfw_social_flat_items sfw_strict_unused_social_flat_items
+#define sfw_social_wp_from_pairs sfw_strict_unused_social_wp_from_pairs
 #define sfw_social_lds_bytes sfw_strict_unused_social_lds_bytes
 #define sfw_pair_table_entries sfw_strict_unused_pair_table_entries
 #define sfw_launch_pair_table sfw_strict_unused_launch_pair_table
diff --git a/social_force_window_planner_amd/planner.py b/social_force_window_planner_amd/planner.py
--- a/social_force_window_planner_amd/planner.py
+++ b/social_force_window_planner_amd/planner.py
@@ -85,6 +85,8 @@
         L.sfw_grid_sync.argtypes = [vp]
         L.sfw_grid_fetch.argtypes = [vp, vp, C.POINTER(SfwBest), C.POINTER(SfwBestKey)]
         L.sfw_grid_plan_info.argtypes = [vp, C.POINTER(SfwPlanInfo)]
+        if hasattr(L, "sfw_grid_wp_from_pairs"):
+            L.sfw_grid_wp_from_pairs.argtypes = [vp, C.POINTER(C.c_int32)]
         L.sfw_set_k2_form.argtypes = [vp, C.c_int32]
         L.sfw_set_timing.argtypes = [vp, C.c_int32]
         L.sfw_last_launch_ms.argtypes = [vp, C.c_int32, C.POINTER(C.c_float)]
@@ -439,6 +441,11 @@
         self._check(lib().sfw_grid_plan_info(self._h, C.byref(info)), "sfw_grid_plan_info")
         return info.as_dict()
 
+    def wp_from_pairs(self):
+        on = C.c_int32(0)
+        self._check(lib().sfw_grid_wp_from_pairs(self._h, C.byref(on)), "sfw_grid_wp_from_pairs")
+        return bool(on.value)
+
     def set_k2_form(self, form):
         self._check(lib().sfw_set_k2_form(self._h, form), "sfw_set_k2_form")
 
```

After: 7.671 million (median of 6 runs). 1.0% higher.
